# Lcrypto/mod-interleaveavx_multithreads-FAID

Hardware: AMD Instinct MI355X
Metric: decoded Gb/s @ 10 iters, 50G-PON LDPC; FER match vs AVX512 ref (higher is better)
Workload: dtype i8

## Files before the change

include/lnsfaid.h:

```cpp
#ifndef LNSFAID_H
#define LNSFAID_H

#include <stddef.h>
#include <stdint.h>

#ifdef __cplusplus
extern "C" {
#endif

#define LNSFAID_GROUP 32

#define LNSFAID_OK 0
#define LNSFAID_E_INVAL (-1)
#define LNSFAID_E_CODE (-2)
#define LNSFAID_E_NOMEM (-3)
#define LNSFAID_E_HIP (-4)
#define LNSFAID_E_NODEVICE (-5)
#define LNSFAID_E_INTERNAL (-6)

typedef struct lnsfaid_code {
    int32_t n_var;
    int32_t n_check;
    int32_t n_edges;
    int32_t z;
    int32_t puncture_tail;
    int32_t nb_degres;
    const int32_t* deg;
    const int32_t* deg_rows;
    const uint16_t* pos_vn;
} lnsfaid_code;

typedef struct lnsfaid_cfg {
    int32_t decode_method;
    int32_t max_iteration;
    int32_t factor_1;
    int32_t factor_2;
    int32_t floor_err_count;
    int32_t floor_iter_thresh;
    int32_t ef_elimination;
    int32_t max_bf_iter;
    int32_t bf_L0;
    int32_t bf_L1;
    int32_t bf_alpha;
    int32_t bf_delta;
    int32_t regular_col_weight;
    int32_t hard2_threshold;
    int32_t bf_vote_cap;
    int8_t v2c_map[6][4][8];
    int8_t v2c_map_ef[6][4][8];
} lnsfaid_cfg;

typedef struct lnsfaid_group_stats {
    int32_t iterations;
    int32_t bf_iterations;
} lnsfaid_group_stats;

typedef struct lnsfaid_codeword_stats {
    int32_t iterations;
    int32_t bf_iterations;
    int32_t unsatisfied;
} lnsfaid_codeword_stats;

typedef struct lnsfaid_ctx lnsfaid_ctx;


int lnsfaid_code_50gpon(lnsfaid_code* code, uint16_t* pos_vn, int32_t* deg3, int32_t* deg_rows3);

int lnsfaid_cfg_default(lnsfaid_cfg* cfg, int32_t decode_method, int32_t max_iteration);

#define LNSFAID_TABLES_FAID3 0
#define LNSFAID_TABLES_FAID32 1
#define LNSFAID_TABLES_FAID2 2
int lnsfaid_cfg_table_preset(lnsfaid_cfg* cfg, int32_t preset);

int lnsfaid_cfg_ef_elimination(lnsfaid_cfg* cfg, int32_t mode);


int lnsfaid_create(lnsfaid_ctx** ctx, const lnsfaid_code* code, const lnsfaid_cfg* cfg,
                   int32_t device, size_t max_groups);
void lnsfaid_destroy(lnsfaid_ctx* ctx);

int lnsfaid_set_cfg(lnsfaid_ctx* ctx, const lnsfaid_cfg* cfg);


int lnsfaid_decode(lnsfaid_ctx* ctx, const int8_t* fixInput, size_t n_groups,
                   int8_t* decodedBits, lnsfaid_group_stats* stats);

int lnsfaid_decode_device(lnsfaid_ctx* ctx, const int8_t* d_fixInput, size_t n_groups,
                          int8_t* d_decodedBits, lnsfaid_group_stats* d_stats);

#define LNSFAID_STOP_GROUP 0
#define LNSFAID_STOP_CODEWORD 1
int lnsfaid_set_early_stop(lnsfaid_ctx* ctx, int32_t rule);
int lnsfaid_early_stop(const lnsfaid_ctx* ctx);
int lnsfaid_decode_codewords(lnsfaid_ctx* ctx, const int8_t* fixInput, size_t n_groups, int8_t* decodedBits,
                             lnsfaid_codeword_stats* cw_stats);
int lnsfaid_decode_codewords_device(lnsfaid_ctx* ctx, const int8_t* d_fixInput, size_t n_groups, int8_t* d_decodedBits,
                                    lnsfaid_codeword_stats* d_cw_stats);

int lnsfaid_count_errors(lnsfaid_ctx* ctx, const int8_t* decodedBits, const int8_t* inputBits,
                         size_t n_groups, uint64_t out[4]);
int lnsfaid_count_errors_device(lnsfaid_ctx* ctx, const int8_t* d_decodedBits,
                                const int8_t* d_inputBits, size_t n_groups, uint64_t out[4]);

int lnsfaid_decode_packed(lnsfaid_ctx* ctx, const uint8_t* llr4, size_t n_groups, uint32_t* bits, lnsfaid_group_stats* stats);
int lnsfaid_decode_packed_device(lnsfaid_ctx* ctx, const uint8_t* d_llr4, size_t n_groups, uint32_t* d_bits,
                                 lnsfaid_group_stats* d_stats);
int lnsfaid_decode_codewords_packed(lnsfaid_ctx* ctx, const uint8_t* llr4, size_t n_groups, uint32_t* bits,
                                    lnsfaid_codeword_stats* cw_stats);
int lnsfaid_decode_codewords_packed_device(lnsfaid_ctx* ctx, const uint8_t* d_llr4, size_t n_groups, uint32_t* d_bits,
                                           lnsfaid_codeword_stats* d_cw_stats);
int lnsfaid_count_errors_packed(lnsfaid_ctx* ctx, const uint32_t* bits, const uint8_t* msg, size_t n_groups, uint64_t out[4]);
int lnsfaid_count_errors_packed_device(lnsfaid_ctx* ctx, const uint32_t* d_bits, const uint8_t* d_msg, size_t n_groups,
                                       uint64_t out[4]);
int lnsfaid_pack_llr4(const int8_t* fixInput, size_t n_values, uint8_t* llr4);
int lnsfaid_unpack_bits(const uint32_t* bits, size_t n_bits, int8_t* decodedBits);
int lnsfaid_pack_bits(const int8_t* inputBits, size_t n_bits, uint8_t* packed);


int lnsfaid_frontend_device(lnsfaid_ctx* ctx, const uint32_t* seeds, const uint64_t* draws_before, size_t n_streams,
                            int32_t mod_type, float sigma, float scale, const int8_t* codeword, int8_t* d_fixInput);
int lnsfaid_frontend_device_states(lnsfaid_ctx* ctx, const uint32_t* states, const uint64_t* draws_before, size_t n_streams,
                                   int32_t mod_type, float sigma, float scale, const int8_t* codeword, int8_t* d_fixInput);
uint64_t lnsfaid_frontend_draws_per_group(const lnsfaid_ctx* ctx, int32_t mod_type);

int lnsfaid_frontend_set_exact(lnsfaid_ctx* ctx, int32_t exact);
int lnsfaid_frontend_fastpath_bounds(lnsfaid_ctx* ctx, double measured[2], double assumed[2]);

int lnsfaid_frontend_set_interleave(lnsfaid_ctx* ctx, int32_t interleave_mod_type);

int lnsfaid_frontend_set_frames(lnsfaid_ctx* ctx, const int8_t* outputBits, const int8_t* inputBits, size_t n_streams);
int lnsfaid_frontend_input_bits(lnsfaid_ctx* ctx, const int8_t** d_inputBits);

int lnsfaid_demap_device(lnsfaid_ctx* ctx, const float* d_rx, size_t n_groups, int32_t mod_type, float scale, int8_t* d_fixInput);
int lnsfaid_demap_packed_device(lnsfaid_ctx* ctx, const float* d_rx, size_t n_groups, int32_t mod_type, float scale, uint8_t* d_llr4);
int lnsfaid_demap_host(int32_t n_var, int32_t n_check, int32_t interleave_mod_type, const float* rx, size_t n_groups,
                       int32_t mod_type, float scale, int8_t* fixInput);
int lnsfaid_demap_packed_host(int32_t n_var, int32_t n_check, int32_t interleave_mod_type, const float* rx, size_t n_groups,
                              int32_t mod_type, float scale, uint8_t* llr4);


int lnsfaid_code_parity_inverse(const lnsfaid_code* code, uint8_t* circ, size_t bytes);

int lnsfaid_encode_device(lnsfaid_ctx* ctx, const int8_t* d_inputBits, size_t n_groups, int8_t* d_outputBits);
int lnsfaid_encode(lnsfaid_ctx* ctx, const int8_t* inputBits, size_t n_groups, int8_t* outputBits);

int lnsfaid_frontend_random_frames(lnsfaid_ctx* ctx, const uint64_t* keys, size_t n_streams);

int lnsfaid_io_buffers(lnsfaid_ctx* ctx, int8_t** d_fixInput, int8_t** d_decodedBits, lnsfaid_group_stats** d_stats);

int lnsfaid_host_register(void* ptr, size_t bytes);
int lnsfaid_host_unregister(void* ptr);

int lnsfaid_read_stats(lnsfaid_ctx* ctx, lnsfaid_group_stats* stats, size_t n_groups);

#define LNSFAID_COMM_ID_BYTES 128
int lnsfaid_comm_unique_id(uint8_t id[LNSFAID_COMM_ID_BYTES]);
int lnsfaid_comm_init(lnsfaid_ctx* ctx, int32_t n_ranks, int32_t rank, const uint8_t id[LNSFAID_COMM_ID_BYTES]);
int lnsfaid_comm_attach(lnsfaid_ctx* ctx, void* nccl_comm);
int lnsfaid_comm_destroy(lnsfaid_ctx* ctx);
int lnsfaid_allreduce_counters(lnsfaid_ctx* ctx, uint64_t counters[4]);

int lnsfaid_select_kernel(lnsfaid_ctx* ctx, int32_t rows_per_lane);
int lnsfaid_kernel_rows_per_lane(const lnsfaid_ctx* ctx);

int lnsfaid_select_waves(lnsfaid_ctx* ctx, int32_t waves_per_codeword);
int lnsfaid_kernel_waves(const lnsfaid_ctx* ctx);

#define LNSFAID_MSG_REGISTERS 1
#define LNSFAID_MSG_HBM 2
int lnsfaid_select_message_store(lnsfaid_ctx* ctx, int32_t where);
int lnsfaid_message_store(const lnsfaid_ctx* ctx);

#define LNSFAID_ZERO_SHIFT_ON 1
#define LNSFAID_ZERO_SHIFT_OFF 2
int lnsfaid_select_zero_shift(lnsfaid_ctx* ctx, int32_t mode);
int lnsfaid_zero_shift_groups(const lnsfaid_ctx* ctx, int32_t* groups, int32_t n);
int lnsfaid_code_zero_shift_order(const lnsfaid_code* code, int32_t* groups, int32_t* order);

int lnsfaid_kernel_residency(lnsfaid_ctx* ctx, int32_t* workgroups_per_cu, int32_t* lds_limit);


int lnsfaid_kernel_time(lnsfaid_ctx* ctx, double* out_ms, uint64_t* out_launches, int32_t reset);

void* lnsfaid_stream(lnsfaid_ctx* ctx);

const char* lnsfaid_strerror(int err);
const char* lnsfaid_last_hip_error(void);
const char* lnsfaid_version(void);

#ifdef __cplusplus
}
#endif
#endif
```

mod-interleaveavx_multithreads-faid_amd/csrc/lnsfaid_capi.hip:

```cpp
#include <hip/hip_runtime.h>

#include <dlfcn.h>
#include <rccl/rccl.h>

#include <cstdio>
#include <cstdlib>
#include <cstring>
#include <new>
#include <vector>

#include "lnsfaid_device.h"
#include "lnsfaid_quantise.h"
#include "lnsfaid_swar.h"

extern "C" hipError_t lf_launch_decode(int method, int uniform_w, const LfKernelArgs* args, size_t lds_bytes,
                                       hipStream_t stream);
extern "C" const void* lf_decode_func(int method, int uniform_w);
extern "C" int lf_decode_threads(void);
extern "C" const void* lf_decode4_func(int method, int ef, int rm);
extern "C" int lf_decode4_threads(void);
extern "C" hipError_t lf_launch_decode4(int method, int ef, int rm, const LfKernelArgs* args, size_t lds_bytes, hipStream_t stream);
extern "C" int lf_decode4_rm_layers(void);
extern "C" const void* lf_decode4cw_func(int method, int ef, int rm);
extern "C" hipError_t lf_launch_decode4cw(int method, int ef, int rm, const LfCwArgs* args, size_t lds_bytes, hipStream_t stream);
extern "C" const void* lf_decode4p_func(int method, int ef, int rm, int per_codeword);
extern "C" hipError_t lf_launch_decode4p(int method, int ef, int rm, const LfKernelArgs* args, size_t lds_bytes, hipStream_t stream);
extern "C" hipError_t lf_launch_decode4pcw(int method, int ef, int rm, const LfCwArgs* args, size_t lds_bytes, hipStream_t stream);
extern "C" hipError_t lf_launch_unpack_llr4(const uint8_t* d_llr4, int8_t* d_fix, size_t n_values, hipStream_t stream);
extern "C" hipError_t lf_launch_pack_bits(const int8_t* d_decoded, uint32_t* d_bits, size_t n_values, hipStream_t stream);
extern "C" hipError_t lf_launch_count_errors_packed(const uint32_t* d_bits, const uint32_t* d_msg, int n_var, int k_info, size_t n_cw,
                                                    unsigned long long* out, hipStream_t stream);
extern "C" int lf_decode4z_inst(int deg, int zg);
extern "C" const void* lf_decode4z_func(int method);
extern "C" hipError_t lf_launch_decode4z(int method, const LfKernelArgs* args, size_t lds_bytes, hipStream_t stream);
extern "C" const void* lf_decode5_func(int method);
extern "C" int lf_decode5_threads(void);
extern "C" hipError_t lf_launch_decode5(int method, const LfKernelArgs* args, size_t lds_bytes, hipStream_t stream);
extern "C" hipError_t lf_launch_count_errors(const int8_t* decoded, const int8_t* input_bits, int n_var, int k_info,
                                             size_t n_cw, unsigned long long* out, hipStream_t stream);

extern "C" hipError_t lf_launch_frontend(const uint32_t* d_seeds, const unsigned long long* d_draws, int n_streams, int mod_type,
                                         float sigma_ch, float scale, const int8_t* d_codeword, const int8_t* d_frames, int n_var,
                                         int n_check, int interleave, int fast, int8_t* d_fix, hipStream_t stream);
extern "C" hipError_t lf_launch_demap(const float* d_rx, size_t n_groups, int mod_type, float scale, int n_var, int n_check,
                                      int interleave, int packed, void* d_out, hipStream_t stream);
extern "C" hipError_t lf_frontend_fastpath_scan(double* d_out2, hipStream_t stream);
extern "C" void lf_frontend_fastpath_assumed(double* eps2);
extern "C" hipError_t lf_launch_encode(const LfDevCode* d_code, int n_check, const uint32_t* d_bsup, const uint32_t* d_bsup_off,
                                       const int8_t* d_in, const unsigned long long* d_keys, size_t n_groups, int8_t* d_out,
                                       int8_t* d_info, hipStream_t stream);

#include <atomic>
#include <chrono>
#include <condition_variable>
#include <mutex>
#include <thread>
struct LfCombiner;
static thread_local char g_hip_err[256] = "";
static std::atomic<int> g_live_contexts(0);
#define LF_SPIN_CONTEXTS 4
static bool sync_blocking()
{
    static const char* e = getenv("LNSFAID_SYNC");
    if (e && e[0] == 's') return false;
    if (e && e[0] == 'b') return true;
    return g_live_contexts.load(std::memory_order_relaxed) > LF_SPIN_CONTEXTS;
}

static int hip_fail(hipError_t e, const char* what)
{
    snprintf(g_hip_err, sizeof(g_hip_err), "%s: %s", what, hipGetErrorString(e));
    return LNSFAID_E_HIP;
}
#define HIP_TRY(call)                                      \
    do {                                                   \
        hipError_t e_ = (call);                            \
        if (e_ != hipSuccess) return hip_fail(e_, #call);  \
    } while (0)

#define LF_IO_CHUNKS 8
#define LF_MAX_CHAIN 6

struct lnsfaid_ctx {
    int device = 0;
    size_t max_groups = 0;
    LfDevCode hcode;
    LfDevCfg hcfg;
    int n_var = 0, n_check = 0, k_info = 0;
    size_t lds_bytes = 0;
    hipStream_t stream = nullptr;
    hipEvent_t ev0 = nullptr, ev1 = nullptr;
    hipEvent_t ev_chain[LF_MAX_CHAIN + 1] = {};
    hipEvent_t ev_block = nullptr;
    uint32_t slot_seen[LF_MAX_CHAIN] = {};
    int predicted_launches = 1;
    hipStream_t s_in = nullptr, s_out = nullptr;
    hipEvent_t ev_in[LF_IO_CHUNKS] = {};
    LfDevCode* d_code = nullptr;
    LfDevCfg* d_cfg = nullptr;
    int8_t* d_en = nullptr;
    uint4* d_rows = nullptr;
    uint32_t* d_bits = nullptr;
    LfLaneState* d_lane = nullptr;
    int32_t* d_status[2] = { nullptr, nullptr };
    uint32_t* d_remaining = nullptr;
    int32_t* d_live = nullptr;
    unsigned long long* d_counters = nullptr;
    uint32_t* h_remaining = nullptr;
    unsigned long long* h_counters = nullptr;
    int8_t* d_io_in = nullptr;
    int8_t* d_io_out = nullptr;
    lnsfaid_group_stats* d_io_stats = nullptr;
    lnsfaid_codeword_stats* d_io_cw_stats = nullptr;
    uint8_t* d_pk_in = nullptr;
    uint32_t* d_pk_out = nullptr;
    lnsfaid_group_stats* d_pk_stats = nullptr;
    int early_stop = LNSFAID_STOP_GROUP;
    int rows_per_lane = 0;
    int waves_per_cw = 0;
    int msg_store = 0;
    int zero_shift = 0;
    struct LfCombiner* comb = nullptr;
    int comb_slot = -1;
    const void* checked_fn[4] = {};
    int resident_wg[4] = {}, lds_wg[4] = {};
    void* comm = nullptr;
    bool comm_owned = false;
    unsigned long long* d_reduce = nullptr;
    double kernel_ms = 0.0;
    uint64_t kernel_launches = 0;
    uint32_t* d_fe_seeds = nullptr;
    unsigned long long* d_fe_draws = nullptr;
    int8_t* d_fe_codeword = nullptr;
    int8_t* d_fe_frames = nullptr;
    int8_t* d_fe_input = nullptr;
    size_t fe_frames_streams = 0;
    int fe_interleave = 1;
    int fe_exact = 0;
    int enc_state = 0;
    uint32_t* d_enc_sup = nullptr;
    uint32_t* d_enc_off = nullptr;
    unsigned long long* d_fe_keys = nullptr;
};

static int stream_wait(lnsfaid_ctx* ctx)
{
    if (sync_blocking()) {
        HIP_TRY(hipEventRecord(ctx->ev_block, ctx->stream));
        HIP_TRY(hipEventSynchronize(ctx->ev_block));
    } else {
        HIP_TRY(hipStreamSynchronize(ctx->stream));
    }
    return LNSFAID_OK;
}

static int weight_class(int w) { return w == 3 ? 0 : (w == 6 ? 1 : (w == 11 ? 2 : 3)); }

static int build_code(const lnsfaid_code* code, LfDevCode* out)
{
    memset(out, 0, sizeof(*out));
    if (!code || !code->pos_vn || !code->deg || !code->deg_rows) return LNSFAID_E_INVAL;
    const int Z = code->z, N = code->n_var, M = code->n_check, E = code->n_edges;
    if (Z != LF_Z) return LNSFAID_E_CODE;
    if (N <= 0 || M <= 0 || N % Z || M % Z || M >= N) return LNSFAID_E_CODE;
    const int nbr = M / Z, nbc = N / Z, K = N - M;
    if (nbr > LF_MAX_BR || nbc > LF_MAX_BC) return LNSFAID_E_CODE;
    if (K % 4 || M % 4 || N % LF_T) return LNSFAID_E_CODE;
    if (code->puncture_tail < 0 || code->puncture_tail > N) return LNSFAID_E_CODE;
    std::vector<int> row_deg;
    row_deg.reserve(M);
    long e_total = 0;
    for (int k = 0; k < code->nb_degres; ++k) {
        if (code->deg_rows[k] < 0 || code->deg[k] < 2 || code->deg[k] > LF_MAX_DEG) return LNSFAID_E_CODE;
        for (int i = 0; i < code->deg_rows[k]; ++i) { row_deg.push_back(code->deg[k]); e_total += code->deg[k]; }
    }
    if ((int)row_deg.size() != M || e_total != E) return LNSFAID_E_CODE;

    size_t e = 0;
    for (int br = 0; br < nbr; ++br) {
        const int deg = row_deg[(size_t)br * Z];
        out->deg[br] = deg;
        const uint16_t* row0 = code->pos_vn + e;
        for (int j = 0; j < 64; ++j) out->sbtab[br][j] = 0u;
        for (int j = 0; j < 32; ++j) out->sbplain[br][j] = 0u;
        int prev_cb = -1;
        for (int j = 0; j < deg; ++j) {
            const int cb = row0[j] / Z, sh = row0[j] % Z;
            if (row0[j] >= N || cb <= prev_cb) return LNSFAID_E_CODE;
            prev_cb = cb;
            out->circ[br][j].sb = (uint32_t)cb * (uint32_t)Z + (uint32_t)sh;
            out->sbtab[br][LF_JCODE_A(j)] = out->sbtab[br][LF_JCODE_B(j)] = out->circ[br][j].sb;
            out->sbplain[br][j] = (((uint32_t)cb * (uint32_t)Z) << 16) | (((uint32_t)sh) << 2);
            out->s4tab[br][j] = ((uint32_t)sh) << 2;
            out->cbtab[br][j] = (uint32_t)cb * (uint32_t)Z;
            if (out->col_weight[cb] >= LF_MAX_COLW) return LNSFAID_E_CODE;
            out->colcirc[cb][out->col_weight[cb]++] = (uint32_t)br | ((uint32_t)sh << 8);
        }
        for (int i = 0; i < Z; ++i) {
            if (row_deg[(size_t)br * Z + i] != deg) return LNSFAID_E_CODE;
            for (int j = 0; j < deg; ++j) {
                const uint32_t sb = out->circ[br][j].sb;
                const int want = (int)(sb / (uint32_t)Z * (uint32_t)Z + (sb % (uint32_t)Z + (uint32_t)i) % (uint32_t)Z);
                if (code->pos_vn[e + (size_t)i * deg + j] != want) return LNSFAID_E_CODE;
            }
        }
        e += (size_t)deg * Z;
        for (int j = 0; j < 32; ++j) out->zsbplain[br][j] = 0u;
        int n = 0;
        for (int zero = 1; zero >= 0; --zero)
            for (int j = 0; j < deg; ++j)
                if ((out->s4tab[br][j] == 0u) == (zero != 0)) {
                    out->zsbplain[br][n] = out->sbplain[br][j];
                    out->zs4tab[br][n] = out->s4tab[br][j];
                    out->zcbtab[br][n] = out->cbtab[br][j];
                    ++n;
                }
        int n_zero = 0;
        while (n_zero < deg && out->zs4tab[br][n_zero] == 0u) ++n_zero;
        out->zinst[br] = lf_decode4z_inst(deg, n_zero / 4);
    }
    {
        const int nw = N / 32, pw = M / 32;
        const uint32_t hard0 = lf_lds_off_hard(N), zero = lf_lds_off_zero(N, nw, pw);
        if (lf_lds_bytes(N, nw, pw) > 0xffffu) return LNSFAID_E_CODE;
        for (int br = 0; br < LF_MAX_BR; ++br)
            for (int j = 0; j < LF_MAX_DEG; ++j)
                for (int k = 0; k < 8; ++k) {
                    uint2 e; e.x = zero | (zero << 16); e.y = 0;
                    if (br < nbr && j < out->deg[br]) {
                        const uint32_t sb = out->circ[br][j].sb, cb = sb / (uint32_t)Z, sh = sb % (uint32_t)Z;
                        const uint32_t o = (32u * (uint32_t)k + sh) & 255u, q = o >> 5;
                        e.x = (hard0 + 4u * (cb * 8u + q)) | ((hard0 + 4u * (cb * 8u + ((q + 1u) & 7u))) << 16);
                        e.y = o & 31u;
                    }
                    out->synw[br][j][k] = e;
                }
    }
    for (int br = 0; br < nbr; ++br)
        for (int j = 0; j < out->deg[br]; ++j)
            out->circ[br][j].wclass = (uint32_t)weight_class(out->col_weight[out->circ[br][j].sb / (uint32_t)Z]);
    out->n_var = N; out->n_check = M; out->k_info = K; out->nbr = nbr; out->nbc = nbc;
    out->puncture_tail = code->puncture_tail;
    out->n_words = N / 32; out->p_words = M / 32;
    return LNSFAID_OK;
}

static void build_wcols(LfDevCode* code, int W)
{
    code->n_wcols = 0;
    for (int cb = 0; cb < code->nbc; ++cb)
        if (code->col_weight[cb] == W) code->wcol[code->n_wcols++] = cb;
    bool seen[LF_MAX_BC] = {};
    for (int br = 0; br < LF_MAX_BR; ++br) {
        code->era_edges[br] = 0;
        for (int j = 0; br < code->nbr && j < code->deg[br]; ++j) {
            const int cb = (int)(code->circ[br][j].sb / LF_Z);
            if (code->col_weight[cb] == W && !seen[cb]) { seen[cb] = true; code->era_edges[br] |= 1u << j; }
        }
    }
}

static int build_cfg(const lnsfaid_cfg* cfg, LfDevCfg* out)
{
    if (!cfg) return LNSFAID_E_INVAL;
    if (cfg->decode_method < 0 || cfg->decode_method > 5) return LNSFAID_E_INVAL;
    if (cfg->max_iteration < 0 || cfg->max_iteration > (1 << 20)) return LNSFAID_E_INVAL;
    if (cfg->max_bf_iter < 0 || cfg->max_bf_iter > (1 << 20)) return LNSFAID_E_INVAL;
    if (cfg->regular_col_weight < 0 || cfg->regular_col_weight > LF_MAX_COLW) return LNSFAID_E_INVAL;
    memset(out, 0, sizeof(*out));
    out->method = cfg->decode_method;
    out->max_iter = cfg->max_iteration;
    out->factor_1 = cfg->decode_method == 0 ? (int16_t)cfg->factor_1 : (int8_t)cfg->factor_1;
    out->factor_2 = cfg->decode_method == 0 ? (int16_t)cfg->factor_2 : (int8_t)cfg->factor_2;
    out->floor_err_count = cfg->floor_err_count;
    out->floor_iter_thresh = cfg->floor_iter_thresh;
    out->ef = cfg->ef_elimination;
    out->max_bf = (cfg->decode_method == 0 || cfg->decode_method == 1) ? 0 : cfg->max_bf_iter;
    out->L0 = cfg->bf_L0; out->L1 = cfg->bf_L1; out->alpha = cfg->bf_alpha; out->delta = cfg->bf_delta;
    out->W = cfg->regular_col_weight;
    out->hard2_thr = cfg->hard2_threshold;
    out->vote_cap = (int8_t)cfg->bf_vote_cap;
    if ((cfg->decode_method == 1 || cfg->decode_method == 3 || cfg->decode_method == 4)
        && ((int8_t)cfg->factor_1 < 0 || (int8_t)cfg->factor_2 < 1)) return LNSFAID_E_INVAL;
    if (cfg->decode_method == 5 && cfg->ef_elimination != 1) return LNSFAID_E_INVAL;
    if (cfg->decode_method == 2 && (cfg->ef_elimination < 0 || cfg->ef_elimination > 2)) return LNSFAID_E_INVAL;
    if (cfg->decode_method != 2 && cfg->decode_method != 5 && cfg->ef_elimination != 0) return LNSFAID_E_INVAL;
    out->uniform_w = 1;
    for (int it = 0; it < 6; ++it)
        for (int w = 0; w < 4; ++w) {
            for (int a = 0; a < 8; ++a) {
                const int v = cfg->v2c_map[it][w][a], ve = cfg->v2c_map_ef[it][w][a];
                if ((cfg->decode_method == 2 || cfg->decode_method == 5) && (v < 0 || v > 7)) return LNSFAID_E_INVAL;
                if ((cfg->decode_method == 5 || cfg->ef_elimination >= 1) && (ve < 0 || ve > 7)) return LNSFAID_E_INVAL;
                uint32_t* l = a < 4 ? &out->lut_lo[it][w] : &out->lut_hi[it][w];
                uint32_t* le = a < 4 ? &out->lut_ef_lo[it][w] : &out->lut_ef_hi[it][w];
                *l |= (uint32_t)(v & 0xff) << (8 * (a & 3));
                *le |= (uint32_t)(ve & 0xff) << (8 * (a & 3));
                if (a > 0 && (v < cfg->v2c_map[it][w][a - 1] || ((cfg->decode_method == 5 || cfg->ef_elimination >= 1) && ve < cfg->v2c_map_ef[it][w][a - 1])))
                    out->uniform_w = 0;
            }
            if (out->lut_lo[it][w] != out->lut_lo[it][0] || out->lut_hi[it][w] != out->lut_hi[it][0]) out->uniform_w = 0;
            if ((cfg->decode_method == 5 || cfg->ef_elimination >= 1)
                && (out->lut_ef_lo[it][w] != out->lut_ef_lo[it][0] || out->lut_ef_hi[it][w] != out->lut_ef_hi[it][0]))
                out->uniform_w = 0;
        }
    if (cfg->decode_method == 0) {
        out->uniform_w = (out->factor_1 == out->factor_2) ? 1 : 0;
        out->nms_fits = sw_nms_fits(out->factor_1, out->factor_2) ? 1 : 0;
        if (out->nms_fits) sw_nms_tables(out->factor_1, out->nms_t);
    }
    if (cfg->decode_method == 2 && cfg->ef_elimination >= 1 && !out->uniform_w) return LNSFAID_E_INVAL;
    out->bf_fast = (out->W == 3 && ((int8_t)out->alpha == 0 || (int8_t)out->alpha == 1)) ? 1 : 0;
    return LNSFAID_OK;
}

static int check_code_for_method(const LfDevCode* code, int method)
{
    if (method == 3)
        for (int cb = 0; cb < code->nbc; ++cb)
            if (code->col_weight[cb] > 15) return LNSFAID_E_CODE;
    return LNSFAID_OK;
}

extern "C" int lnsfaid_comm_destroy(lnsfaid_ctx* ctx);
static int comb_join(lnsfaid_ctx* ctx);
static void comb_leave(lnsfaid_ctx* ctx, int slot);
extern "C" void lnsfaid_destroy(lnsfaid_ctx* ctx)
{
    if (!ctx) return;
    if (ctx->comb_slot >= 0) { comb_leave(ctx, ctx->comb_slot); ctx->comb_slot = -1; }
    g_live_contexts.fetch_sub(1, std::memory_order_relaxed);
    (void)hipSetDevice(ctx->device);
    if (ctx->stream) (void)hipStreamSynchronize(ctx->stream);
    (void)lnsfaid_comm_destroy(ctx);
    (void)hipFree(ctx->d_reduce);
    (void)hipFree(ctx->d_code); (void)hipFree(ctx->d_cfg); (void)hipFree(ctx->d_en); (void)hipFree(ctx->d_rows);
    (void)hipFree(ctx->d_bits); (void)hipFree(ctx->d_lane); (void)hipFree(ctx->d_status[0]); (void)hipFree(ctx->d_status[1]);
    (void)hipFree(ctx->d_remaining); (void)hipFree(ctx->d_live); (void)hipFree(ctx->d_counters);
    (void)hipFree(ctx->d_io_in); (void)hipFree(ctx->d_io_out); (void)hipFree(ctx->d_io_stats);
    (void)hipFree(ctx->d_io_cw_stats);
    (void)hipFree(ctx->d_pk_in); (void)hipFree(ctx->d_pk_out); (void)hipFree(ctx->d_pk_stats);
    (void)hipFree(ctx->d_fe_seeds); (void)hipFree(ctx->d_fe_draws); (void)hipFree(ctx->d_fe_codeword);
    (void)hipFree(ctx->d_fe_frames); (void)hipFree(ctx->d_fe_input);
    (void)hipFree(ctx->d_enc_sup); (void)hipFree(ctx->d_enc_off); (void)hipFree(ctx->d_fe_keys);
    if (ctx->h_remaining) (void)hipHostFree(ctx->h_remaining);
    if (ctx->h_counters) (void)hipHostFree(ctx->h_counters);
    if (ctx->ev0) (void)hipEventDestroy(ctx->ev0);
    if (ctx->ev1) (void)hipEventDestroy(ctx->ev1);
    for (auto e : ctx->ev_chain) if (e) (void)hipEventDestroy(e);
    if (ctx->ev_block) (void)hipEventDestroy(ctx->ev_block);
    if (ctx->stream) (void)hipStreamDestroy(ctx->stream);
    if (ctx->s_in) (void)hipStreamDestroy(ctx->s_in);
    if (ctx->s_out) (void)hipStreamDestroy(ctx->s_out);
    for (auto e : ctx->ev_in) if (e) (void)hipEventDestroy(e);
    delete ctx;
}

static int alloc_state(lnsfaid_ctx* ctx);
static int create_impl(lnsfaid_ctx* ctx, const lnsfaid_code* code, const lnsfaid_cfg* cfg)
{
    int rc = build_code(code, &ctx->hcode);
    if (rc) return rc;
    rc = build_cfg(cfg, &ctx->hcfg);
    if (rc) return rc;
    ctx->n_var = ctx->hcode.n_var; ctx->n_check = ctx->hcode.n_check; ctx->k_info = ctx->hcode.k_info;
    rc = check_code_for_method(&ctx->hcode, ctx->hcfg.method);
    if (rc) return rc;
    build_wcols(&ctx->hcode, ctx->hcfg.W);
    return alloc_state(ctx);
}

static int alloc_state(lnsfaid_ctx* ctx)
{
    ctx->n_var = ctx->hcode.n_var; ctx->n_check = ctx->hcode.n_check; ctx->k_info = ctx->hcode.k_info;
    ctx->lds_bytes = lf_lds_bytes(ctx->n_var, ctx->hcode.n_words, ctx->hcode.p_words);
    if (ctx->lds_bytes > 64 * 1024) return LNSFAID_E_CODE;

    int ndev = 0;
    if (hipGetDeviceCount(&ndev) != hipSuccess || ndev <= 0 || ctx->device < 0 || ctx->device >= ndev) {
        snprintf(g_hip_err, sizeof(g_hip_err), "no usable HIP device (count %d, asked for %d)", ndev, ctx->device);
        return LNSFAID_E_NODEVICE;
    }
    HIP_TRY(hipSetDevice(ctx->device));
    HIP_TRY(hipStreamCreateWithFlags(&ctx->stream, hipStreamNonBlocking));
    HIP_TRY(hipEventCreate(&ctx->ev0));
    HIP_TRY(hipEventCreate(&ctx->ev1));
    const size_t n_cw = ctx->max_groups * LNSFAID_GROUP;
    HIP_TRY(hipMalloc(&ctx->d_code, sizeof(LfDevCode)));
    HIP_TRY(hipMalloc(&ctx->d_cfg, sizeof(LfDevCfg)));
    HIP_TRY(hipMalloc(&ctx->d_en, n_cw * (size_t)ctx->n_var));
    HIP_TRY(hipMalloc(&ctx->d_rows, n_cw * (size_t)ctx->hcode.nbr * LF_T * sizeof(uint4)));
    HIP_TRY(hipMalloc(&ctx->d_bits, n_cw * (size_t)3 * ctx->hcode.n_words * sizeof(uint32_t)));
    HIP_TRY(hipMalloc(&ctx->d_lane, n_cw * sizeof(LfLaneState)));
    HIP_TRY(hipMalloc(&ctx->d_status[0], n_cw * sizeof(int32_t)));
    HIP_TRY(hipMalloc(&ctx->d_status[1], n_cw * sizeof(int32_t)));
    HIP_TRY(hipMalloc(&ctx->d_remaining, LF_MAX_CHAIN * sizeof(uint32_t)));
    HIP_TRY(hipMemset(ctx->d_remaining, 0, LF_MAX_CHAIN * sizeof(uint32_t)));
    for (auto& e : ctx->ev_chain) HIP_TRY(hipEventCreate(&e));
    HIP_TRY(hipEventCreateWithFlags(&ctx->ev_block, hipEventBlockingSync | hipEventDisableTiming));
    HIP_TRY(hipMalloc(&ctx->d_live, n_cw * sizeof(int32_t)));
    HIP_TRY(hipMalloc(&ctx->d_counters, 4 * sizeof(unsigned long long)));
    HIP_TRY(hipHostMalloc((void**)&ctx->h_remaining, LF_MAX_CHAIN * sizeof(uint32_t), hipHostMallocDefault));
    HIP_TRY(hipHostMalloc((void**)&ctx->h_counters, 4 * sizeof(unsigned long long), hipHostMallocDefault));
    HIP_TRY(hipMemcpy(ctx->d_code, &ctx->hcode, sizeof(LfDevCode), hipMemcpyHostToDevice));
    HIP_TRY(hipMemcpy(ctx->d_cfg, &ctx->hcfg, sizeof(LfDevCfg), hipMemcpyHostToDevice));
    return LNSFAID_OK;
}

extern "C" int lnsfaid_create(lnsfaid_ctx** out, const lnsfaid_code* code, const lnsfaid_cfg* cfg, int32_t device,
                              size_t max_groups)
{
    if (!out || !code || !cfg || max_groups == 0 || max_groups > ((size_t)1 << 24)) return LNSFAID_E_INVAL;
    *out = nullptr;
    lnsfaid_ctx* ctx = new (std::nothrow) lnsfaid_ctx();
    if (!ctx) return LNSFAID_E_NOMEM;
    ctx->device = device;
    ctx->max_groups = max_groups;
    if (const char* e = getenv("LNSFAID_ROWS_PER_LANE"))
        ctx->rows_per_lane = (e[0] == '2') ? 2 : 0;
    if (const char* e = getenv("LNSFAID_WAVES_PER_CODEWORD"))
        ctx->waves_per_cw = (e[0] == '2') ? 2 : 0;
    if (const char* e = getenv("LNSFAID_FRONTEND_EXACT"))
        ctx->fe_exact = (e[0] == '1') ? 1 : 0;
    if (const char* e = getenv("LNSFAID_MSG_STORE"))
        ctx->msg_store = (e[0] == 'h') ? LNSFAID_MSG_HBM : ((e[0] == 'r') ? LNSFAID_MSG_REGISTERS : 0);
    if (const char* e = getenv("LNSFAID_ZERO_SHIFT"))
        ctx->zero_shift = (e[0] == 'o' && e[1] == 'f') ? LNSFAID_ZERO_SHIFT_OFF : 0;
    g_live_contexts.fetch_add(1, std::memory_order_relaxed);
    const int rc = create_impl(ctx, code, cfg);
    if (rc) { lnsfaid_destroy(ctx); return rc; }
    ctx->comb_slot = comb_join(ctx);
    *out = ctx;
    return LNSFAID_OK;
}

extern "C" int lnsfaid_set_cfg(lnsfaid_ctx* ctx, const lnsfaid_cfg* cfg)
{
    if (!ctx || !cfg) return LNSFAID_E_INVAL;
    LfDevCfg n;
    int rc = build_cfg(cfg, &n);
    if (rc) return rc;
    rc = check_code_for_method(&ctx->hcode, n.method);
    if (rc) return rc;
    if (memcmp(&n, &ctx->hcfg, sizeof(n)) == 0) return LNSFAID_OK;
    HIP_TRY(hipSetDevice(ctx->device));
    HIP_TRY(hipStreamSynchronize(ctx->stream));
    if (n.W != ctx->hcfg.W) {
        build_wcols(&ctx->hcode, n.W);
        HIP_TRY(hipMemcpy(ctx->d_code, &ctx->hcode, sizeof(LfDevCode), hipMemcpyHostToDevice));
    }
    ctx->hcfg = n;
    HIP_TRY(hipMemcpy(ctx->d_cfg, &ctx->hcfg, sizeof(LfDevCfg), hipMemcpyHostToDevice));
    return LNSFAID_OK;
}

static void apply_devcfg(lnsfaid_ctx* ctx, const LfDevCfg& n)
{
    (void)hipStreamSynchronize(ctx->stream);
    ctx->hcfg = n;
    (void)hipMemcpy(ctx->d_cfg, &ctx->hcfg, sizeof(LfDevCfg), hipMemcpyHostToDevice);
}

static bool kernel4_possible(const lnsfaid_ctx* ctx)
{
    const int m = ctx->hcfg.method;
    if (m < 0 || m > 5) return false;
    if (m == 0) return ctx->hcfg.nms_fits != 0;
    if ((m == 2 || m == 5) && !ctx->hcfg.uniform_w) return false;
    return true;
}
static bool use_kernel4(const lnsfaid_ctx* ctx)
{
    if (ctx->hcfg.method == 2 && ctx->hcfg.ef >= 1) return true;
    if (ctx->rows_per_lane == 2) return false;
    return kernel4_possible(ctx);
}

extern "C" int lnsfaid_select_kernel(lnsfaid_ctx* ctx, int32_t rows_per_lane)
{
    if (!ctx || (rows_per_lane != 0 && rows_per_lane != 2 && rows_per_lane != 4)) return LNSFAID_E_INVAL;
    if (rows_per_lane == 4 && !kernel4_possible(ctx)) return LNSFAID_E_INVAL;
    if (rows_per_lane == 2 && ctx->hcfg.method == 2 && ctx->hcfg.ef >= 1) return LNSFAID_E_INVAL;
    ctx->rows_per_lane = rows_per_lane;
    return LNSFAID_OK;
}

extern "C" int lnsfaid_kernel_rows_per_lane(const lnsfaid_ctx* ctx) { return ctx ? (use_kernel4(ctx) ? 4 : 2) : LNSFAID_E_INVAL; }

static bool kernel5_possible(const lnsfaid_ctx* ctx)
{
    const int m = ctx->hcfg.method;
    return kernel4_possible(ctx) && m >= 1 && m <= 5 && !(m == 2 && ctx->hcfg.ef == 2) && ctx->hcode.n_words >= 7 * 64;
}
static bool use_kernel5(const lnsfaid_ctx* ctx) { return ctx->waves_per_cw == 2 && use_kernel4(ctx) && kernel5_possible(ctx); }

extern "C" int lnsfaid_select_waves(lnsfaid_ctx* ctx, int32_t waves_per_codeword)
{
    if (!ctx || waves_per_codeword < 0 || waves_per_codeword > 2) return LNSFAID_E_INVAL;
    if (waves_per_codeword == 2 && !(use_kernel4(ctx) && kernel5_possible(ctx))) return LNSFAID_E_INVAL;
    ctx->waves_per_cw = waves_per_codeword;
    return LNSFAID_OK;
}

extern "C" int lnsfaid_kernel_waves(const lnsfaid_ctx* ctx) { return ctx ? (use_kernel5(ctx) ? 2 : 1) : LNSFAID_E_INVAL; }

static bool msg_registers_possible(const lnsfaid_ctx* ctx)
{
    if (ctx->hcfg.method == 0) return false;
    return ctx->hcode.nbr <= lf_decode4_rm_layers() && !(ctx->hcfg.method == 2 && ctx->hcfg.ef == 2);
}
static bool use_msg_registers(const lnsfaid_ctx* ctx)
{
    if (!msg_registers_possible(ctx) || use_kernel5(ctx)) return false;
    return ctx->msg_store != LNSFAID_MSG_HBM;
}

static int layer_zero_groups(const lnsfaid_ctx* ctx, int br) { return (ctx->hcode.zinst[br] >> 8) & 0xff; }
static bool zero_shift_possible(const lnsfaid_ctx* ctx)
{
    if (!use_kernel4(ctx) || use_kernel5(ctx) || !use_msg_registers(ctx)) return false;
    if (ctx->hcfg.method < 1 || ctx->hcfg.method > 5 || !lf_decode4z_func(ctx->hcfg.method)) return false;
    for (int br = 0; br < ctx->hcode.nbr; ++br)
        if (layer_zero_groups(ctx, br) >= 1) return true;
    return false;
}
static bool use_zero_shift(const lnsfaid_ctx* ctx) { return ctx->zero_shift != LNSFAID_ZERO_SHIFT_OFF && zero_shift_possible(ctx); }

extern "C" int lnsfaid_select_zero_shift(lnsfaid_ctx* ctx, int32_t mode)
{
    if (!ctx || mode < 0 || mode > LNSFAID_ZERO_SHIFT_OFF) return LNSFAID_E_INVAL;
    if (mode == LNSFAID_ZERO_SHIFT_ON && !zero_shift_possible(ctx)) return LNSFAID_E_INVAL;
    ctx->zero_shift = mode;
    return LNSFAID_OK;
}

extern "C" int lnsfaid_zero_shift_groups(const lnsfaid_ctx* ctx, int32_t* groups, int32_t n)
{
    if (!ctx || n < 0 || (n > 0 && !groups)) return LNSFAID_E_INVAL;
    const bool on = use_zero_shift(ctx);
    for (int br = 0; br < n; ++br) groups[br] = (on && br < ctx->hcode.nbr) ? layer_zero_groups(ctx, br) : 0;
    return on ? 1 : 0;
}

extern "C" int lnsfaid_code_zero_shift_order(const lnsfaid_code* code, int32_t* groups, int32_t* order)
{
    LfDevCode* dc = new (std::nothrow) LfDevCode;
    if (!dc) return LNSFAID_E_NOMEM;
    const int rc = build_code(code, dc);
    if (rc) { delete dc; return rc; }
    const int nbr = dc->nbr;
    for (int br = 0; br < nbr; ++br) {
        int n_zero = 0;
        while (n_zero < dc->deg[br] && dc->zs4tab[br][n_zero] == 0u) ++n_zero;
        if (groups) groups[br] = n_zero / 4;
        for (int j = 0; order && j < LF_MAX_DEG; ++j) {
            order[br * LF_MAX_DEG + j] = -1;
            for (int i = 0; j < dc->deg[br] && i < dc->deg[br]; ++i)
                if (dc->cbtab[br][i] == dc->zcbtab[br][j] && dc->s4tab[br][i] == dc->zs4tab[br][j]) order[br * LF_MAX_DEG + j] = i;
        }
    }
    delete dc;
    return nbr;
}

static bool cw_possible(const lnsfaid_ctx* ctx) { return ctx->waves_per_cw != 2 && use_kernel4(ctx); }

static bool packed_kernel(const lnsfaid_ctx* ctx) { return use_kernel4(ctx) && !use_kernel5(ctx); }

static const void* selected_kernel(const lnsfaid_ctx* ctx, int* threads, int rule, bool packed = false)
{
    if (packed) {
        *threads = lf_decode4_threads();
        return lf_decode4p_func(ctx->hcfg.method, ctx->hcfg.ef, use_msg_registers(ctx) ? 1 : 0, rule == LNSFAID_STOP_CODEWORD ? 1 : 0);
    }
    if (rule == LNSFAID_STOP_CODEWORD) {
        *threads = lf_decode4_threads();
        return cw_possible(ctx) ? lf_decode4cw_func(ctx->hcfg.method, ctx->hcfg.ef, use_msg_registers(ctx) ? 1 : 0) : nullptr;
    }
    if (use_kernel5(ctx)) {
        *threads = lf_decode5_threads();
        return lf_decode5_func(ctx->hcfg.method);
    }
    if (use_zero_shift(ctx)) {
        *threads = lf_decode4_threads();
        return lf_decode4z_func(ctx->hcfg.method);
    }
    if (use_kernel4(ctx)) {
        *threads = lf_decode4_threads();
        return lf_decode4_func(ctx->hcfg.method, ctx->hcfg.ef, use_msg_registers(ctx) ? 1 : 0);
    }
    *threads = lf_decode_threads();
    return lf_decode_func(ctx->hcfg.method, ctx->hcfg.uniform_w);
}

extern "C" int lnsfaid_select_message_store(lnsfaid_ctx* ctx, int32_t where)
{
    if (!ctx || where < 0 || where > LNSFAID_MSG_HBM) return LNSFAID_E_INVAL;
    if (where == LNSFAID_MSG_REGISTERS && !msg_registers_possible(ctx)) return LNSFAID_E_INVAL;
    ctx->msg_store = where;
    return LNSFAID_OK;
}

extern "C" int lnsfaid_message_store(const lnsfaid_ctx* ctx)
{
    if (!ctx) return LNSFAID_E_INVAL;
    if (!use_kernel4(ctx)) return LNSFAID_MSG_HBM;
    return use_msg_registers(ctx) ? LNSFAID_MSG_REGISTERS : LNSFAID_MSG_HBM;
}

static int kernel_check(lnsfaid_ctx* ctx, int rule, bool packed = false)
{
    int threads = 0;
    const void* fn = selected_kernel(ctx, &threads, rule, packed);
    if (!fn) return rule == LNSFAID_STOP_CODEWORD ? LNSFAID_E_INVAL : LNSFAID_E_INTERNAL;
    const int slot = rule + (packed ? 2 : 0);
    if (fn == ctx->checked_fn[slot]) return LNSFAID_OK;
    hipFuncAttributes at;
    HIP_TRY(hipFuncGetAttributes(&at, fn));
    if (at.sharedSizeBytes != 0) {
        snprintf(g_hip_err, sizeof(g_hip_err), "decode kernel has %zu bytes of static LDS: its En image would not start at LDS offset 0",
                 (size_t)at.sharedSizeBytes);
        return LNSFAID_E_INTERNAL;
    }
    int wg = 0;
    HIP_TRY(hipOccupancyMaxActiveBlocksPerMultiprocessor(&wg, fn, threads, ctx->lds_bytes));
    hipDeviceProp_t prop;
    HIP_TRY(hipGetDeviceProperties(&prop, ctx->device));
    const size_t lds_cu = prop.maxSharedMemoryPerMultiProcessor ? prop.maxSharedMemoryPerMultiProcessor : 160 * 1024;
    const size_t gran = 512;
    int by_lds = (int)(lds_cu / ((ctx->lds_bytes + gran - 1) / gran * gran));
    const int by_waves = 32 / ((threads + 63) / 64);
    if (by_lds > by_waves) by_lds = by_waves;
    ctx->checked_fn[slot] = fn; ctx->resident_wg[slot] = wg; ctx->lds_wg[slot] = by_lds;
    static const bool trace = getenv("LNSFAID_TRACE") != nullptr;
    if (trace)
        fprintf(stderr, "[lnsfaid] decode kernel: %d threads, %d VGPRs, %zu B LDS per workgroup, %d workgroups per CU (LDS alone: %d)%s\n",
                threads, at.numRegs, ctx->lds_bytes, wg, by_lds, wg < by_lds ? "  ** residency lost **" : "");
    return LNSFAID_OK;
}

extern "C" int lnsfaid_kernel_residency(lnsfaid_ctx* ctx, int32_t* workgroups_per_cu, int32_t* lds_limit)
{
    if (!ctx) return LNSFAID_E_INVAL;
    HIP_TRY(hipSetDevice(ctx->device));
    const int rc = kernel_check(ctx, ctx->early_stop);
    if (rc) return rc;
    if (workgroups_per_cu) *workgroups_per_cu = ctx->resident_wg[ctx->early_stop];
    if (lds_limit) *lds_limit = ctx->lds_wg[ctx->early_stop];
    return LNSFAID_OK;
}

static int decode_device_impl(lnsfaid_ctx* ctx, const int8_t* d_fixInput, size_t n_groups, int8_t* d_decodedBits,
                              lnsfaid_group_stats* d_stats, bool status_preloaded, bool packed = false);
static int decode_cw_device_impl(lnsfaid_ctx* ctx, const int8_t* d_fixInput, size_t n_groups, int8_t* d_decodedBits,
                                 lnsfaid_group_stats* d_stats, lnsfaid_codeword_stats* d_cw_stats, bool status_preloaded,
                                 bool packed = false);
static int decode_device_rule(lnsfaid_ctx* ctx, const int8_t* d_fixInput, size_t n_groups, int8_t* d_decodedBits, lnsfaid_group_stats* d_stats,
                              lnsfaid_codeword_stats* d_cw_stats, int rule, bool status_preloaded)
{
    if (rule == LNSFAID_STOP_CODEWORD)
        return decode_cw_device_impl(ctx, d_fixInput, n_groups, d_decodedBits, d_stats, d_cw_stats, status_preloaded);
    return decode_device_impl(ctx, d_fixInput, n_groups, d_decodedBits, d_stats, status_preloaded);
}
extern "C" int lnsfaid_decode_device(lnsfaid_ctx* ctx, const int8_t* d_fixInput, size_t n_groups, int8_t* d_decodedBits,
                                     lnsfaid_group_stats* d_stats)
{
    if (!ctx) return LNSFAID_E_INVAL;
    return decode_device_rule(ctx, d_fixInput, n_groups, d_decodedBits, d_stats, nullptr, ctx->early_stop, false);
}
extern "C" int lnsfaid_decode_codewords_device(lnsfaid_ctx* ctx, const int8_t* d_fixInput, size_t n_groups, int8_t* d_decodedBits,
                                               lnsfaid_codeword_stats* d_cw_stats)
{
    return decode_cw_device_impl(ctx, d_fixInput, n_groups, d_decodedBits, nullptr, d_cw_stats, false);
}

extern "C" int lnsfaid_set_early_stop(lnsfaid_ctx* ctx, int32_t rule)
{
    if (!ctx || (rule != LNSFAID_STOP_GROUP && rule != LNSFAID_STOP_CODEWORD)) return LNSFAID_E_INVAL;
    ctx->early_stop = rule;
    return LNSFAID_OK;
}
extern "C" int lnsfaid_early_stop(const lnsfaid_ctx* ctx) { return ctx ? ctx->early_stop : LNSFAID_E_INVAL; }

static int decode_cw_device_impl(lnsfaid_ctx* ctx, const int8_t* d_fixInput, size_t n_groups, int8_t* d_decodedBits,
                                 lnsfaid_group_stats* d_stats, lnsfaid_codeword_stats* d_cw_stats, bool status_preloaded, bool packed)
{
    if (!ctx || (n_groups && (!d_fixInput || !d_decodedBits))) return LNSFAID_E_INVAL;
    if (n_groups > ctx->max_groups) return LNSFAID_E_INVAL;
    if (!cw_possible(ctx)) return LNSFAID_E_INVAL;
    if (n_groups == 0) return LNSFAID_OK;
    HIP_TRY(hipSetDevice(ctx->device));
    {
        const int rc = kernel_check(ctx, LNSFAID_STOP_CODEWORD, packed);
        if (rc) return rc;
    }
    const size_t n_cw = n_groups * LNSFAID_GROUP;
    LfCwArgs a;
    a.code = ctx->d_code; a.cfg = ctx->d_cfg;
    a.fix_input = d_fixInput; a.decoded = d_decodedBits;
    a.st_rows = ctx->d_rows;
    a.skip = status_preloaded ? ctx->d_status[0] : nullptr;
    a.stats = d_stats; a.cw_stats = d_cw_stats; a.n_cw = (int32_t)n_cw;
    if (d_stats) HIP_TRY(hipMemsetAsync(d_stats, 0, n_groups * sizeof(lnsfaid_group_stats), ctx->stream));
    static const bool trace = getenv("LNSFAID_TRACE") != nullptr;
    HIP_TRY(hipEventRecord(ctx->ev_chain[0], ctx->stream));
    if (packed) HIP_TRY(lf_launch_decode4pcw(ctx->hcfg.method, ctx->hcfg.ef, use_msg_registers(ctx) ? 1 : 0, &a, ctx->lds_bytes, ctx->stream));
    else HIP_TRY(lf_launch_decode4cw(ctx->hcfg.method, ctx->hcfg.ef, use_msg_registers(ctx) ? 1 : 0, &a, ctx->lds_bytes, ctx->stream));
    HIP_TRY(hipEventRecord(ctx->ev_chain[1], ctx->stream));
    { const int rcw = stream_wait(ctx); if (rcw) return rcw; }
    float ms = 0.f;
    HIP_TRY(hipEventElapsedTime(&ms, ctx->ev_chain[0], ctx->ev_chain[1]));
    ctx->kernel_ms += ms;
    ctx->kernel_launches += 1;
    if (trace) fprintf(stderr, "[lnsfaid] per-codeword launch: %.3f ms, %zu codewords\n", ms, n_cw);
    return LNSFAID_OK;
}

static int decode_device_impl(lnsfaid_ctx* ctx, const int8_t* d_fixInput, size_t n_groups, int8_t* d_decodedBits,
                              lnsfaid_group_stats* d_stats, bool status_preloaded, bool packed)
{
    if (!ctx || (n_groups && (!d_fixInput || !d_decodedBits))) return LNSFAID_E_INVAL;
    if (n_groups > ctx->max_groups) return LNSFAID_E_INVAL;
    if (n_groups == 0) return LNSFAID_OK;
    HIP_TRY(hipSetDevice(ctx->device));
    {
        const int rc = kernel_check(ctx, LNSFAID_STOP_GROUP, packed);
        if (rc) return rc;
    }
    const size_t n_cw = n_groups * LNSFAID_GROUP;
#ifdef LF4_LIVE_PROOF
    HIP_TRY(hipMemsetAsync(ctx->d_live, 0, n_cw * sizeof(int32_t), ctx->stream));
#endif

    LfKernelArgs a;
    a.code = ctx->d_code; a.cfg = ctx->d_cfg;
    a.fix_input = d_fixInput; a.decoded = d_decodedBits;
    a.st_en = ctx->d_en; a.st_rows = ctx->d_rows; a.st_bits = ctx->d_bits; a.st_lane = ctx->d_lane;
    a.live = ctx->d_live; a.stats = d_stats; a.n_cw = (int32_t)n_cw;

    const long max_launches = 2L * ((long)ctx->hcfg.max_iter + ctx->hcfg.max_bf + 2) + 2 + LF_MAX_CHAIN;
    static const bool trace = getenv("LNSFAID_TRACE") != nullptr;
    int cur = 0;
    long launch = 0, needed = 0;
    bool done = false;
    while (!done) {
        if (launch >= max_launches) return LNSFAID_E_INTERNAL;
        int chain = launch == 0 ? ctx->predicted_launches : 1;
        if (chain < 1) chain = 1;
        if (chain > LF_MAX_CHAIN) chain = LF_MAX_CHAIN;
        for (int j = 0; j < chain; ++j) {
            a.status_cur = (launch + j == 0 && !status_preloaded) ? nullptr : ctx->d_status[cur];
            a.status_next = ctx->d_status[cur ^ 1];
            a.remaining = ctx->d_remaining + j;
            HIP_TRY(hipEventRecord(ctx->ev_chain[j], ctx->stream));
            if (packed) HIP_TRY(lf_launch_decode4p(ctx->hcfg.method, ctx->hcfg.ef, use_msg_registers(ctx) ? 1 : 0, &a, ctx->lds_bytes, ctx->stream));
            else if (use_kernel5(ctx)) HIP_TRY(lf_launch_decode5(ctx->hcfg.method, &a, ctx->lds_bytes, ctx->stream));
            else if (use_zero_shift(ctx)) HIP_TRY(lf_launch_decode4z(ctx->hcfg.method, &a, ctx->lds_bytes, ctx->stream));
            else if (use_kernel4(ctx)) HIP_TRY(lf_launch_decode4(ctx->hcfg.method, ctx->hcfg.ef, use_msg_registers(ctx) ? 1 : 0, &a, ctx->lds_bytes, ctx->stream));
            else HIP_TRY(lf_launch_decode(ctx->hcfg.method, ctx->hcfg.uniform_w, &a, ctx->lds_bytes, ctx->stream));
            cur ^= 1;
        }
        HIP_TRY(hipEventRecord(ctx->ev_chain[chain], ctx->stream));
        HIP_TRY(hipMemcpyAsync(ctx->h_remaining, ctx->d_remaining, (size_t)chain * sizeof(uint32_t), hipMemcpyDeviceToHost, ctx->stream));
        { const int rcw = stream_wait(ctx); if (rcw) return rcw; }
        for (int j = 0; j < chain; ++j) {
            const uint32_t left = ctx->h_remaining[j] - ctx->slot_seen[j];
            ctx->slot_seen[j] = ctx->h_remaining[j];
            float ms = 0.f;
            HIP_TRY(hipEventElapsedTime(&ms, ctx->ev_chain[j], ctx->ev_chain[j + 1]));
            ctx->kernel_ms += ms;
            ctx->kernel_launches += 1;
            if (trace) fprintf(stderr, "[lnsfaid] launch %ld: %.3f ms, %u codewords left%s\n", launch + j, ms, left, done ? " (queued ahead, batch already complete)" : "");
            if (!done && left == 0) { done = true; needed = launch + j + 1; }
        }
        launch += chain;
    }
    ctx->predicted_launches = (int)needed;
    return LNSFAID_OK;
}

static int ensure_io(lnsfaid_ctx* ctx)
{
    if (ctx->d_io_in) return LNSFAID_OK;
    const size_t bytes = ctx->max_groups * LNSFAID_GROUP * (size_t)ctx->n_var;
    HIP_TRY(hipMalloc(&ctx->d_io_in, bytes));
    HIP_TRY(hipMalloc(&ctx->d_io_out, bytes));
    HIP_TRY(hipMalloc(&ctx->d_io_stats, ctx->max_groups * sizeof(lnsfaid_group_stats)));
    return LNSFAID_OK;
}

#define LF_COMB_SLOTS 128
#define LF_COMB_QUIET_US 150
#define LF_COMB_WINDOW_US 1500
#define LF_COMB_DEVICES 16
#define LF_COMB_WORKERS 4
#define LF_COMB_MIN_MEMBERS 4
enum { LF_SLOT_FREE = 0, LF_SLOT_IDLE, LF_SLOT_PENDING, LF_SLOT_RUNNING, LF_SLOT_DONE };
struct LfSlot {
    int state = LF_SLOT_FREE;
    int rc = 0;
    LfDevCfg cfg;
    int rule = LNSFAID_STOP_GROUP;
    lnsfaid_group_stats stats;
};
struct LfCombiner {
    int device = 0;
    std::mutex m;
    std::condition_variable cv_work, cv_done;
    std::thread worker[LF_COMB_WORKERS];
    bool stop = false, dead = false;
    bool gathering = false;
    int running = 0;
    lnsfaid_ctx* pool[LF_COMB_WORKERS] = {};
    LfDevCode code;
    size_t group_bytes = 0;
    int8_t *h_in = nullptr, *h_out = nullptr;
    int8_t *d_in_map = nullptr, *d_out_map = nullptr;
    int32_t* h_status = nullptr;
    lnsfaid_group_stats* h_stats = nullptr;
    LfSlot slots[LF_COMB_SLOTS];
    int members = 0, pending = 0;
    char err[256] = "";
    uint64_t batches = 0, calls = 0;
    double gather_ms = 0, device_ms = 0;
};
static std::mutex g_comb_mutex;
static LfCombiner* g_comb[LF_COMB_DEVICES] = {};

static int comb_workers()
{
    static const int n = [] {
        const char* e = getenv("LNSFAID_COMB_WORKERS");
        const int v = e ? atoi(e) : 2;
        return v < 1 ? 1 : (v > LF_COMB_WORKERS ? LF_COMB_WORKERS : v);
    }();
    return n;
}

static int comb_batches()
{
    static const int v = [] {
        const char* e = getenv("LNSFAID_COMB_BATCHES");
        const int n = e ? atoi(e) : 0;
        return n > 64 ? 64 : n;
    }();
    return v > comb_workers() ? v : comb_workers();
}

static bool comb_enabled()
{
    static const char* e = getenv("LNSFAID_COALESCE");
    return !(e && e[0] == '0');
}

static void apply_devcfg(lnsfaid_ctx* ctx, const LfDevCfg& n);

static void comb_run_batch(LfCombiner* cb, int w, const int* batch, int nb)
{
    lnsfaid_ctx* P = cb->pool[w];
    int32_t* h_status = cb->h_status + (size_t)w * LF_COMB_SLOTS * LNSFAID_GROUP;
    lnsfaid_group_stats* h_stats = cb->h_stats + (size_t)w * LF_COMB_SLOTS;
    int rc = LNSFAID_OK;
    auto fail = [&](hipError_t e, const char* what) { if (rc == LNSFAID_OK && e != hipSuccess) rc = hip_fail(e, what); };
    int lo = LF_COMB_SLOTS, hi = -1;
    for (int i = 0; i < nb; ++i) { lo = batch[i] < lo ? batch[i] : lo; hi = batch[i] > hi ? batch[i] : hi; }
    const size_t n = (size_t)hi + 1;
    for (size_t g = 0; g < n; ++g) {
        bool active = false;
        for (int i = 0; i < nb; ++i) active = active || (size_t)batch[i] == g;
        for (int l = 0; l < LNSFAID_GROUP; ++l) h_status[g * LNSFAID_GROUP + l] = active ? 0 : LF_DONE;
    }
    fail(hipSetDevice(cb->device), "hipSetDevice");
    if (rc == LNSFAID_OK && memcmp(&P->hcfg, &cb->slots[batch[0]].cfg, sizeof(LfDevCfg)) != 0) apply_devcfg(P, cb->slots[batch[0]].cfg);
    const size_t gb = cb->group_bytes, span = (size_t)(hi - lo + 1);
    fail(hipMemcpyAsync(P->d_status[0], h_status, n * LNSFAID_GROUP * sizeof(int32_t), hipMemcpyHostToDevice, P->stream), "status upload");
    static const bool copy_mode = getenv("LNSFAID_COMB_COPY") != nullptr;
    const int8_t* k_in = cb->d_in_map;
    int8_t* k_out = cb->d_out_map;
    if (copy_mode || !k_in || !k_out) {
        fail(hipMemcpyAsync(P->d_io_in + (size_t)lo * gb, cb->h_in + (size_t)lo * gb, span * gb, hipMemcpyHostToDevice, P->stream), "fixInput upload");
        k_in = P->d_io_in; k_out = P->d_io_out;
    }
    if (rc == LNSFAID_OK) rc = decode_device_rule(P, k_in, n, k_out, P->d_io_stats, nullptr, cb->slots[batch[0]].rule, true);
    if (rc == LNSFAID_OK) {
        if (k_out == P->d_io_out)
            fail(hipMemcpyAsync(cb->h_out + (size_t)lo * gb, P->d_io_out + (size_t)lo * gb, span * gb, hipMemcpyDeviceToHost, P->stream), "decodedBits download");
        fail(hipMemcpyAsync(h_stats + lo, P->d_io_stats + lo, span * sizeof(lnsfaid_group_stats), hipMemcpyDeviceToHost, P->stream), "stats download");
        if (rc == LNSFAID_OK) rc = stream_wait(P);
    }
    std::lock_guard<std::mutex> lk(cb->m);
    if (rc != LNSFAID_OK) snprintf(cb->err, sizeof(cb->err), "%s", g_hip_err);
    for (int i = 0; i < nb; ++i) {
        LfSlot& s = cb->slots[batch[i]];
        s.rc = rc;
        s.stats = h_stats[batch[i]];
        s.state = LF_SLOT_DONE;
    }
    cb->running -= nb;
    cb->batches += 1; cb->calls += (uint64_t)nb;
    cb->cv_done.notify_all();
    cb->cv_work.notify_all();
}

static void comb_worker(LfCombiner* cb, int w)
{
    std::unique_lock<std::mutex> lk(cb->m);
    for (;;) {
        cb->cv_work.wait(lk, [&] { return cb->stop || (cb->pending > 0 && !cb->gathering); });
        if (cb->stop) break;
        cb->gathering = true;
        const auto t_first = std::chrono::steady_clock::now();
        const auto deadline = t_first + std::chrono::microseconds(LF_COMB_WINDOW_US);
        for (;;) {
            const int share = (cb->members + comb_batches() - 1) / comb_batches();
            if (cb->stop || cb->pending >= share || cb->pending + cb->running >= cb->members) break;
            const int seen = cb->pending, seen_running = cb->running;
            auto quiet = std::chrono::steady_clock::now() + std::chrono::microseconds(LF_COMB_QUIET_US);
            if (quiet > deadline) quiet = deadline;
            cb->cv_work.wait_until(lk, quiet, [&] { return cb->pending != seen || cb->running != seen_running || cb->stop; });
            if (cb->pending == seen && cb->running == seen_running) break;
        }
        if (cb->stop) { cb->gathering = false; break; }
        cb->gather_ms += std::chrono::duration<double, std::milli>(std::chrono::steady_clock::now() - t_first).count();
        int batch[LF_COMB_SLOTS], nb = 0;
        const int cap = cb->members > 8 * comb_workers() ? (cb->members + comb_batches() - 1) / comb_batches() : LF_COMB_SLOTS;
        const LfDevCfg* cfg = nullptr;
        int rule = LNSFAID_STOP_GROUP;
        for (int i = 0; i < LF_COMB_SLOTS && nb < cap; ++i) {
            LfSlot& s = cb->slots[i];
            if (s.state != LF_SLOT_PENDING) continue;
            if (!cfg) { cfg = &s.cfg; rule = s.rule; }
            if (memcmp(cfg, &s.cfg, sizeof(LfDevCfg)) != 0 || s.rule != rule) continue;
            s.state = LF_SLOT_RUNNING;
            batch[nb++] = i;
        }
        cb->pending -= nb;
        cb->running += nb;
        cb->gathering = false;
        cb->cv_work.notify_all();
        if (nb == 0) continue;
        if (!cb->pool[w]) {
            lk.unlock();
            int rc = LNSFAID_OK;
            lnsfaid_ctx* P = new (std::nothrow) lnsfaid_ctx();
            if (!P) rc = LNSFAID_E_NOMEM;
            if (!rc) {
                P->device = cb->device; P->max_groups = LF_COMB_SLOTS;
                P->hcode = cb->code; P->hcfg = cb->slots[batch[0]].cfg;
                g_live_contexts.fetch_add(1, std::memory_order_relaxed);
                rc = alloc_state(P);
                if (!rc) rc = ensure_io(P);
                if (rc) { lnsfaid_destroy(P); P = nullptr; }
            }
            lk.lock();
            if (rc) {
                cb->dead = true;
                for (int i = 0; i < nb; ++i) { cb->slots[batch[i]].rc = rc; cb->slots[batch[i]].state = LF_SLOT_DONE; }
                cb->running -= nb;
                cb->cv_done.notify_all();
                continue;
            }
            cb->pool[w] = P;
        }
        lk.unlock();
        const auto t_dev = std::chrono::steady_clock::now();
        comb_run_batch(cb, w, batch, nb);
        lk.lock();
        cb->device_ms += std::chrono::duration<double, std::milli>(std::chrono::steady_clock::now() - t_dev).count();
    }
}

static int comb_join(lnsfaid_ctx* ctx)
{
    if (!comb_enabled() || ctx->max_groups != 1 || ctx->device < 0 || ctx->device >= LF_COMB_DEVICES) return -1;
    std::lock_guard<std::mutex> g(g_comb_mutex);
    LfCombiner* cb = g_comb[ctx->device];
    if (!cb) {
        cb = new (std::nothrow) LfCombiner();
        if (!cb) return -1;
        cb->device = ctx->device;
        cb->code = ctx->hcode;
        cb->group_bytes = (size_t)LNSFAID_GROUP * (size_t)ctx->n_var;
        g_comb[ctx->device] = cb;
    }
    std::lock_guard<std::mutex> lk(cb->m);
    if (cb->dead || memcmp(&cb->code, &ctx->hcode, sizeof(LfDevCode)) != 0) return -1;
    if (cb->members >= 1 && !cb->h_in) {
        const size_t bytes = (size_t)LF_COMB_SLOTS * cb->group_bytes;
        if (hipSetDevice(cb->device) != hipSuccess
            || hipHostMalloc((void**)&cb->h_in, bytes, hipHostMallocMapped) != hipSuccess
            || hipHostMalloc((void**)&cb->h_out, bytes, hipHostMallocMapped) != hipSuccess
            || hipHostMalloc((void**)&cb->h_status, (size_t)LF_COMB_WORKERS * LF_COMB_SLOTS * LNSFAID_GROUP * sizeof(int32_t), hipHostMallocDefault) != hipSuccess
            || hipHostMalloc((void**)&cb->h_stats, (size_t)LF_COMB_WORKERS * LF_COMB_SLOTS * sizeof(lnsfaid_group_stats), hipHostMallocDefault) != hipSuccess) {
            (void)hipGetLastError();
            if (cb->h_in) (void)hipHostFree(cb->h_in);
            if (cb->h_out) (void)hipHostFree(cb->h_out);
            if (cb->h_status) (void)hipHostFree(cb->h_status);
            if (cb->h_stats) (void)hipHostFree(cb->h_stats);
            cb->h_in = cb->h_out = nullptr; cb->h_status = nullptr; cb->h_stats = nullptr;
            cb->dead = true;
            return -1;
        }
        if (hipHostGetDevicePointer((void**)&cb->d_in_map, cb->h_in, 0) != hipSuccess
            || hipHostGetDevicePointer((void**)&cb->d_out_map, cb->h_out, 0) != hipSuccess) {
            (void)hipGetLastError();
            cb->d_in_map = cb->d_out_map = nullptr;
        }
        for (int w = 0; w < comb_workers(); ++w) cb->worker[w] = std::thread(comb_worker, cb, w);
    }
    for (int i = 0; i < LF_COMB_SLOTS; ++i)
        if (cb->slots[i].state == LF_SLOT_FREE) { cb->slots[i].state = LF_SLOT_IDLE; cb->members += 1; ctx->comb = cb; return i; }
    return -1;
}

static void comb_leave(lnsfaid_ctx* ctx, int slot)
{
    LfCombiner* cb = nullptr;
    {
        std::lock_guard<std::mutex> g(g_comb_mutex);
        cb = ctx->comb;
        if (!cb) return;
        bool last;
        {
            std::lock_guard<std::mutex> lk(cb->m);
            cb->slots[slot].state = LF_SLOT_FREE;
            cb->members -= 1;
            last = cb->members == 0;
            if (last) cb->stop = true;
            cb->cv_work.notify_all();
        }
        if (!last) return;
        if (g_comb[cb->device] == cb) g_comb[cb->device] = nullptr;
    }
    for (auto& th : cb->worker) if (th.joinable()) th.join();
    static const bool trace = getenv("LNSFAID_TRACE") != nullptr;
    if (trace && cb->batches)
        fprintf(stderr, "[lnsfaid] call combiner of device %d: %llu calls in %llu batches (%.1f per batch); per batch %.3f ms gathering, %.3f ms copies + decode\n",
                cb->device, (unsigned long long)cb->calls, (unsigned long long)cb->batches, (double)cb->calls / (double)cb->batches,
                cb->gather_ms / (double)cb->batches, cb->device_ms / (double)cb->batches);
    for (auto P : cb->pool) if (P) lnsfaid_destroy(P);
    if (cb->h_in) { (void)hipHostFree(cb->h_in); (void)hipHostFree(cb->h_out); (void)hipHostFree(cb->h_status); (void)hipHostFree(cb->h_stats); }
    delete cb;
}

static int comb_decode(lnsfaid_ctx* ctx, const int8_t* fixInput, int8_t* decodedBits, lnsfaid_group_stats* stats, int rule, int* rc_out)
{
    if (ctx->comb_slot < 0 || ctx->rows_per_lane != 0 || ctx->msg_store != 0 || ctx->waves_per_cw != 0 || ctx->zero_shift != 0) return 0;
    LfCombiner* cb = ctx->comb;
    const int slot = ctx->comb_slot;
    {
        std::lock_guard<std::mutex> lk(cb->m);
        if (cb->dead || cb->members < LF_COMB_MIN_MEMBERS || !cb->h_in) return 0;
        if (memcmp(&cb->code, &ctx->hcode, sizeof(LfDevCode)) != 0) return 0;
    }
    memcpy(cb->h_in + (size_t)slot * cb->group_bytes, fixInput, cb->group_bytes);
    int rc;
    {
        std::unique_lock<std::mutex> lk(cb->m);
        LfSlot& s = cb->slots[slot];
// ... 841 lines not shown
```

mod-interleaveavx_multithreads-faid_amd/csrc/lnsfaid_swar.h:

```cpp
#ifndef LNSFAID_SWAR_H
#define LNSFAID_SWAR_H

#include <stdint.h>

#if defined(__HIPCC__)
#define SW_DEV 1
#define SW_FN __device__ __forceinline__
#define SW_HD __host__ __device__ __forceinline__
#else
#define SW_DEV 0
#define SW_FN static inline
#define SW_HD static inline
#endif

#define SW_MAX_DEG 24
#ifndef SW_ILP
#define SW_ILP 4
#endif

#if SW_DEV
#define SW_SCHED_FENCE() __builtin_amdgcn_sched_barrier(0)
#else
#define SW_SCHED_FENCE() ((void)0)
#endif

SW_FN uint32_t sw_perm(uint32_t s0, uint32_t s1, uint32_t sel)
{
#if SW_DEV
    return __builtin_amdgcn_perm(s0, s1, sel);
#else
    const uint64_t in = ((uint64_t)s0 << 32) | s1;
    uint32_t r = 0;
    for (int i = 0; i < 4; ++i) {
        const uint32_t s = (sel >> (8 * i)) & 0xffu;
        uint32_t b;
        if (s >= 13) b = 0xff;
        else if (s == 12) b = 0;
        else if (s >= 8) b = ((in >> (8 * (2 * (s - 8) + 1) + 7)) & 1u) ? 0xffu : 0u;
        else b = (uint32_t)(in >> (8 * s)) & 0xffu;
        r |= b << (8 * i);
    }
    return r;
#endif
}
SW_FN uint32_t sw_alignbyte(uint32_t s0, uint32_t s1, uint32_t s2)
{
#if SW_DEV
    return __builtin_amdgcn_alignbyte(s0, s1, s2);
#else
    const uint64_t in = ((uint64_t)s0 << 32) | s1;
    return (uint32_t)(in >> (8 * (s2 & 3u)));
#endif
}
template <int TT>
SW_FN uint32_t sw_bitop3(uint32_t a, uint32_t b, uint32_t c)
{
#if SW_DEV
    return __builtin_amdgcn_bitop3_b32(a, b, c, TT);
#else
    uint32_t r = 0;
    for (int m = 0; m < 8; ++m)
        if ((TT >> m) & 1) r |= ((m & 4) ? a : ~a) & ((m & 2) ? b : ~b) & ((m & 1) ? c : ~c);
    return r;
#endif
}
#define SW_TT_SEL 0xca
#define SW_TT_XOR3 0x96
#define SW_TT_AND3 0x80
#define SW_TT_ANDOR 0xea
#define SW_TT_NANDOR 0xae
#define SW_TT_A_AND_BORC 0xe0
#define SW_TT_XORAND 0x28
#define SW_TT_BFI_C 0xd8
#define SW_TT_ANDNOT_OR 0xf8
#define SW_TT_XNOR_AND 0x82

SW_FN uint32_t sw_vconst(uint32_t k, uint32_t dep = 0u)
{
#if SW_DEV
    uint32_t r;
    asm("v_mov_b32 %0, %1 ; %2" : "=v"(r) : "s"(k), "s"(dep));
    return r;
#else
    (void)dep;
    return k;
#endif
}

#define SW_T2N_LO 0xf900fafbu
#define SW_T2N_HI 0xf8000000u

struct SwK {
    uint32_t c78, c0642, cfc, sel_sign, tt_lo, tt_hi, oh_lo, oh_hi;
    uint32_t cbit[8];
    uint32_t c7f;
    uint32_t c70;
    uint32_t n_lo, n_hi;
    uint32_t c55, c33, c0f;
    uint32_t cm27;
};
SW_FN SwK sw_consts(uint32_t dep = 0u)
{
    SwK k;
    k.c78 = sw_vconst(0x78787878u, dep); k.c0642 = sw_vconst(0x06040200u, dep); k.cfc = sw_vconst(0xfcu, dep);
    k.sel_sign = sw_vconst(0x0b090a08u, dep);
    k.tt_lo = sw_vconst(0x07030100u, dep); k.tt_hi = sw_vconst(0xff3f1f0fu, dep);
    k.oh_lo = sw_vconst(0x08040201u, dep); k.oh_hi = sw_vconst(0x80402010u, dep);
    for (int e = 0; e < 8; ++e) k.cbit[e] = sw_vconst(0x01010101u << e, dep);
    k.c7f = sw_vconst(0x7f7f7f7fu, dep);
    k.c70 = sw_vconst(0x70707070u, dep);
    k.n_lo = sw_vconst(SW_T2N_LO, dep); k.n_hi = sw_vconst(SW_T2N_HI, dep);
    k.c55 = sw_vconst(0x55555555u, dep); k.c33 = sw_vconst(0x33333333u, dep); k.c0f = sw_vconst(0x0f0f0f0fu, dep);
    k.cm27 = sw_vconst(0u - 0x27272727u, dep);
    return k;
}

SW_FN uint32_t sw_mask7(uint32_t x, uint32_t sel_sign) { return sw_perm(x, x << 8, sel_sign); }
#define SW_SEL_SIGN 0x0b090a08u

SW_FN uint32_t sw_popcount7(uint32_t x)
{
    x &= 0x7f7f7f7fu;
    x = x - ((x >> 1) & 0x55555555u);
    x = (x & 0x33333333u) + ((x >> 2) & 0x33333333u);
    return (x + (x >> 4)) & 0x0f0f0f0fu;
}
SW_FN uint32_t sw_therm2num(uint32_t x, uint32_t n_lo, uint32_t n_hi)
{
    const uint32_t a = sw_perm(n_hi, n_lo, x & 0x0f0f0f0fu);
    const uint32_t b = sw_perm(n_hi, n_lo, (x >> 4) & 0x07070707u);
    return a ^ b;
}
SW_FN uint32_t sw_zero_mask(uint32_t x, uint32_t sel_sign) { return ~sw_mask7(x + 0x7f7f7f7fu, sel_sign); }

SW_FN uint32_t sw_gather4(uint32_t g0, uint32_t g1, uint32_t g2, uint32_t g3)
{
    const uint32_t lo = (g1 << 8) | g0, hi = (g3 << 8) | g2;
    return (hi << 16) | lo;
}
SW_FN uint32_t sw_opaque(uint32_t x)
{
#if SW_DEV
    asm("" : "+v"(x));
#endif
    return x;
}
SW_FN uint32_t sw_node_addr(uint32_t x) { return sw_perm(x, x, 0x0c0c0300u) | ((x >> 8) & 3u); }

SW_FN uint32_t sw_table_pick(uint32_t rowmask, uint32_t w_hi, uint32_t w_lo, uint32_t t_hi, uint32_t t_lo, uint32_t m)
{
    return sw_bitop3<SW_TT_SEL>(rowmask, sw_perm(w_hi, w_lo, m), sw_perm(t_hi, t_lo, m));
}
SW_FN uint32_t sw_word_pick(uint32_t nm3, uint32_t nm4, uint32_t x0, uint32_t x1, uint32_t x2)
{
    return sw_bitop3<SW_TT_SEL>(nm4, sw_bitop3<SW_TT_SEL>(nm3, x0, x1), x2);
}
SW_FN void sw_word_deal(uint32_t keep, uint32_t nm3, uint32_t nm4, uint32_t oh[3])
{
    oh[0] = sw_bitop3<SW_TT_AND3>(keep, nm3, nm4);
    oh[1] = sw_bitop3<0x20>(keep, nm3, nm4);
    oh[2] = keep & ~nm4;
}
SW_FN uint32_t sw_argmin_selector(uint32_t w, uint32_t oh8, uint32_t c7f, uint32_t c01, uint32_t c0642)
{
    return sw_bitop3<SW_TT_ANDOR>(((w & oh8) + c7f) >> 7, c01, c0642);
}

struct SwRow {
    uint32_t x[3];
    uint32_t cw;
    uint32_t pa[2];
};

struct SwParams {
    uint32_t lut_lo, lut_hi;
    uint32_t ef_lo, ef_hi;
    int32_t f1, f2;
    int32_t window;
    int32_t ef_tables;
    uint32_t nms_t[4];
    uint32_t oms_lo[2], oms_hi[2];
};

#if SW_DEV
struct SwLds {
    typedef __attribute__((address_space(3))) uint32_t lds_u32;
    typedef __attribute__((address_space(3))) uint8_t lds_u8;
    SW_FN uint32_t rd32(uint32_t a) const { return *(const lds_u32*)(size_t)a; }
    SW_FN void wr32(uint32_t a, uint32_t v) const { *(lds_u32*)(size_t)a = v; }
    SW_FN uint32_t rd8(uint32_t a) const { return *(const lds_u8*)(size_t)a; }
    SW_FN void wr8(uint32_t a, uint32_t v) const { *(lds_u8*)(size_t)a = (uint8_t)v; }
};
#else
struct SwLds {
    uint8_t* base;
    uint32_t rd32(uint32_t a) const { return (uint32_t)base[a] | ((uint32_t)base[a + 1] << 8) | ((uint32_t)base[a + 2] << 16) | ((uint32_t)base[a + 3] << 24); }
    void wr32(uint32_t a, uint32_t v) const { base[a] = (uint8_t)v; base[a + 1] = (uint8_t)(v >> 8); base[a + 2] = (uint8_t)(v >> 16); base[a + 3] = (uint8_t)(v >> 24); }
    uint32_t rd8(uint32_t a) const { return base[a]; }
    void wr8(uint32_t a, uint32_t v) const { base[a] = (uint8_t)v; }
};
#endif

#define SW_BIAS_EN 120

SW_FN uint32_t sw_en_pos(uint32_t v) { return (v & ~255u) | ((v & 63u) << 2) | ((v >> 6) & 3u); }

#define SW_OMS(M) ((M) == 1 || (M) == 3 || (M) == 4)
#define SW_MINSUM(M) ((M) == 0 || SW_OMS(M))

SW_FN int sw_oms_offset(int x, bool window, bool F, int f1, int f2)
{
    if (window && F) {
        if (x < f2) x += 1;
        if (x <= f1) x += 1;
    } else {
        if (x > f1) x -= 1;
        if (x >= f2) x -= 1;
    }
    return x;
}

SW_FN void sw_oms_tables(SwParams& p)
{
    for (int r = 0; r < 2; ++r) {
        uint32_t lo = 0, hi = 0;
        for (int x = 0; x < 8; ++x) {
            const int a = sw_oms_offset(x, r != 0, r != 0, p.f1, p.f2);
            const uint32_t v = (uint32_t)((a > 7 ? 7 : a) & 0xff);
            if (x < 4) lo |= v << (8 * x); else hi |= v << (8 * (x - 4));
        }
        p.oms_lo[r] = lo; p.oms_hi[r] = hi;
    }
}

SW_HD int sw_nms_cste(int m, int factor)
{
    const uint16_t p = (uint16_t)((uint16_t)m * (uint16_t)(int16_t)factor);
    const int16_t q = (int16_t)(p >> 5);
    const int r = q > 127 ? 127 : q;
    return r > 7 ? 7 : r;
}
SW_HD bool sw_nms_fits(int f1, int f2)
{
    if (f1 != f2) return false;
    for (int m = 1; m < 32; ++m)
        if (sw_nms_cste(m, f1) < sw_nms_cste(m - 1, f1)) return false;
    return sw_nms_cste(15, f1) == 7;
}
SW_HD void sw_nms_tables(int factor, uint32_t nms_t[4])
{
    for (int w = 0; w < 4; ++w) nms_t[w] = 0;
    for (int m = 0; m < 16; ++m) {
        const int c = sw_nms_cste(m, factor);
        const uint32_t code = c >= 7 ? 0xffu : ((1u << c) - 1u);
        nms_t[m >> 2] |= code << (8 * (m & 3));
    }
}

struct SwUpd {
    uint32_t za[2], sb[2];
    uint32_t oc[2], hi[2];
};
template <bool MINSUM, bool FLIP = true>
SW_FN SwUpd sw_update_consts(uint32_t c, uint32_t flip, uint32_t bias)
{
    const uint32_t za_p = 0x1f1f1f1fu - bias, za_n = za_p - c;
    const uint32_t sb_p = 0x27272727u - c, sb_n = 0x27272727u;
    const uint32_t oc_p = 0x3f3f3f3fu - c, oc_n = MINSUM ? 0x3f3f3f3fu : oc_p;
    const uint32_t hi_p = 0xbebebebeu - c, hi_n = MINSUM ? 0xbebebebeu : hi_p;
    SwUpd u;
    if (!FLIP) {
        u.za[1] = za_p; u.za[0] = za_n; u.sb[1] = sb_p; u.sb[0] = sb_n; u.oc[1] = oc_p; u.oc[0] = oc_n; u.hi[1] = hi_p; u.hi[0] = hi_n;
        return u;
    }
    u.za[1] = sw_bitop3<SW_TT_SEL>(flip, za_n, za_p); u.za[0] = sw_bitop3<SW_TT_SEL>(flip, za_p, za_n);
    u.sb[1] = sw_bitop3<SW_TT_SEL>(flip, sb_n, sb_p); u.sb[0] = sw_bitop3<SW_TT_SEL>(flip, sb_p, sb_n);
    if (MINSUM) {
        u.oc[1] = sw_bitop3<SW_TT_SEL>(flip, oc_n, oc_p); u.oc[0] = sw_bitop3<SW_TT_SEL>(flip, oc_p, oc_n);
        u.hi[1] = sw_bitop3<SW_TT_SEL>(flip, hi_n, hi_p); u.hi[0] = sw_bitop3<SW_TT_SEL>(flip, hi_p, hi_n);
    } else {
        u.oc[1] = u.oc[0] = oc_p; u.hi[1] = u.hi[0] = hi_p;
    }
    return u;
}
template <bool MINSUM>
SW_FN uint32_t sw_update(uint32_t tb, uint32_t ms, const SwUpd& u, uint32_t sel_sign, uint32_t c80)
{
    const uint32_t za = sw_bitop3<SW_TT_SEL>(ms, u.za[1], u.za[0]);
    const uint32_t sb = sw_bitop3<SW_TT_SEL>(ms, u.sb[1], u.sb[0]);
    const uint32_t oc = MINSUM ? sw_bitop3<SW_TT_SEL>(ms, u.oc[1], u.oc[0]) : u.oc[1];
    const uint32_t hi = MINSUM ? sw_bitop3<SW_TT_SEL>(ms, u.hi[1], u.hi[0]) : u.hi[1];
    const uint32_t zb = tb + za;
    const uint32_t mo = sw_mask7(zb - oc, sel_sign);
    const uint32_t mq = sw_mask7(zb, sel_sign);
    return sw_bitop3<SW_TT_SEL>(mo, hi, sw_bitop3<SW_TT_SEL>(mq, zb, c80)) - sb;
}

struct SwUpd2 {
    uint32_t c, fm, zc, oc, hi;
};
template <bool MINSUM>
SW_FN SwUpd2 sw_update2_consts(uint32_t c, uint32_t fm, uint32_t bias)
{
    SwUpd2 u;
    u.c = c; u.fm = fm;
    u.zc = 0x1f1f1f1fu - bias - c;
    u.oc = MINSUM ? 0u - 0x3f3f3f3fu : 0x3f3f3f3fu - c;
    u.hi = MINSUM ? 0xbebebebeu : 0xbebebebeu - c;
    return u;
}
SW_FN uint32_t sw_upd2_d(uint32_t ms, const SwUpd2& u) { return sw_bitop3<SW_TT_XORAND>(ms, u.fm, u.c); }
SW_FN uint32_t sw_upd2_zb(uint32_t tb, uint32_t d, const SwUpd2& u) { return tb + d + u.zc; }
template <bool MINSUM>
SW_FN uint32_t sw_upd2_out(uint32_t zb, uint32_t d, const SwUpd2& u)
{
    const uint32_t ov = MINSUM ? zb + d + u.oc : zb - u.oc;
    return sw_bitop3<0xcf>(zb, ov, ov);
}
template <bool MINSUM>
SW_FN uint32_t sw_upd2_limit(uint32_t ms, uint32_t d, const SwUpd2& u, uint32_t c80)
{
    return sw_bitop3<SW_TT_ANDOR>(ms, MINSUM ? u.hi - d : u.hi, c80);
}
SW_FN uint32_t sw_upd2_en(uint32_t mout, uint32_t lim, uint32_t zb, uint32_t d, uint32_t cm27) { return sw_bitop3<SW_TT_SEL>(mout, lim, zb) + d + cm27; }
template <bool MINSUM>
SW_FN uint32_t sw_update2(uint32_t tb, uint32_t ms, const SwUpd2& u, uint32_t sel_sign, uint32_t c80, uint32_t cm27)
{
    const uint32_t d = sw_upd2_d(ms, u);
    const uint32_t zb = sw_upd2_zb(tb, d, u);
    const uint32_t mout = sw_mask7(sw_upd2_out<MINSUM>(zb, d, u), sel_sign);
    return sw_upd2_en(mout, sw_upd2_limit<MINSUM>(ms, d, u, c80), zb, d, cm27);
}

SW_FN void sw_min_edge(uint32_t& t1, uint32_t& t2, uint32_t ta[5], uint32_t u, int j)
{
    t2 = sw_bitop3<SW_TT_A_AND_BORC>(t2, t1, u);
    t1 &= u;
#pragma unroll
    for (int b = 0; b < 5; ++b)
        if (((j >> b) & 1) == (b >= 3 ? 1 : 0)) ta[b] &= u;
}
SW_FN void sw_min_quad(uint32_t& t1, uint32_t& t2, uint32_t ta[5], uint32_t v0, uint32_t v1, uint32_t v2, uint32_t v3, int j0)
{
    const uint32_t p0 = v0 & v1, p1 = v2 & v3, q = p0 & p1;
    const uint32_t o0 = v0 | v1, o1 = v2 | v3;
    const uint32_t m2 = sw_bitop3<SW_TT_A_AND_BORC>(o0, p0, p1);
    const uint32_t y = sw_bitop3<SW_TT_A_AND_BORC>(t2, t1, q);
    t2 = sw_bitop3<SW_TT_AND3>(y, m2, o1);
    t1 &= q;
    ta[0] = sw_bitop3<SW_TT_AND3>(ta[0], v0, v2);
    ta[1] &= p0;
    if (((j0 >> 2) & 1) == 0) ta[2] &= q;
    if (((j0 >> 3) & 1) == 1) ta[3] &= q;
    if (((j0 >> 4) & 1) == 1) ta[4] &= q;
}

SW_FN void sw_sign_edge(uint32_t ns[3], uint32_t ms, int j, uint32_t cbit) { ns[j >> 3] = sw_bitop3<SW_TT_ANDNOT_OR>(ns[j >> 3], ms, cbit); }
template <int NJ>
SW_FN void sw_sign_quad(uint32_t ns[3], const uint32_t* ms, int j0, int deg, bool fixed, uint32_t c55, uint32_t c33, uint32_t c0f)
{
    uint32_t m[4];
#pragma unroll
    for (int g = 0; g < 4; ++g) m[g] = (j0 + g < NJ && (fixed || j0 + g < deg)) ? ms[j0 + g < NJ ? j0 + g : 0] : 0u;
    const bool has1 = j0 + 1 < NJ, has2 = j0 + 2 < NJ, has3 = j0 + 3 < NJ;
    const uint32_t a = has1 ? sw_bitop3<SW_TT_SEL>(c55, m[0], m[1]) : m[0];
    const uint32_t b = has3 ? sw_bitop3<SW_TT_SEL>(c55, m[2], m[3]) : m[2];
    const uint32_t q = has2 ? sw_bitop3<SW_TT_SEL>(c33, a, b) : a;
    ns[j0 >> 3] = (j0 & 4) ? sw_bitop3<SW_TT_SEL>(c0f, ns[j0 >> 3], q) : q;
}

SW_FN uint32_t sw_plane_bit(const SwLds& lds, uint32_t era_plane, uint32_t a)
{
    const uint32_t v = (a & ~255u) | ((a >> 2) & 63u) | ((a & 3u) << 6);
    return (lds.rd32(era_plane + ((v >> 5) << 2)) >> (v & 31u)) & 1u;
}

#if SW_DEV
#define SW_MFN __device__ __forceinline__
#else
#define SW_MFN inline
#endif
struct SwNoXch {
    SW_MFN void put(int, uint32_t) const {}
    SW_MFN uint32_t get(int) const { return 0u; }
    SW_MFN void barrier() const {}
};
#define SW_OWN(j) (WAVES == 1 || (((j) & 1) == WAVE))

template <int METHOD, int DEG, bool ERA = false, int WAVES = 1, int WAVE = 0, int ZG = 0, class Tab, class Xch = SwNoXch>
SW_FN SwRow sw_layer_step(const SwLds& lds, const Tab& tab, const SwParams& p, const SwK& K, uint32_t lane, int deg, SwRow cur, bool fresh,
                          uint32_t rowpar, bool lme, uint32_t era_edges = 0u, uint32_t era_plane = 0u, const Xch& xch = Xch())
{
    static_assert(WAVES == 1 || !ERA, "the erasing variant is built for one wave per codeword only");
    static_assert(!ERA || METHOD == 2, "the erasure exists in Decode_FAID only");
    static_assert(ZG == 0 || (DEG > 0 && WAVES == 1 && !ERA && SW_ILP * ZG <= DEG), "rotation-free groups: per-degree, one-wave, non-erasing instances");
    constexpr int NZ = SW_ILP * ZG;
    constexpr int NJ = DEG > 0 ? DEG : SW_MAX_DEG;
    constexpr bool MINSUM = SW_MINSUM(METHOD);
    constexpr bool QUADS = WAVES == 1 && SW_ILP == 4 && DEG > 0;
    constexpr bool NSTREE = WAVES == 1 && SW_ILP == 4;
    const uint32_t c01 = K.cbit[0], c80 = K.cbit[7], c7f = K.c7f, c78 = K.c78, c0642 = K.c0642, cfc = K.cfc, sel_sign = K.sel_sign;
    const uint32_t tid4 = lane << 2;
    uint32_t s4j[NJ], cbj[NJ];
#pragma unroll
    for (int j = 0; j < NJ; ++j) { s4j[j] = (DEG > 0 || j < deg) ? tab.s4(j) : 0u; cbj[j] = (DEG > 0 || j < deg) ? tab.cb256(j) : 0u; }

    const uint32_t c2o = cur.cw & 0x07070707u, c1o = (cur.cw >> 3) & 0x07070707u;
    const uint32_t kp = 0x08080808u - c2o, kn = 0x08080808u + c2o;
    const uint32_t bias = MINSUM ? 0u : 0x06040200u;
    const uint32_t kt_lo = sw_perm(kn, kp, 0x05010400u) + (MINSUM ? 0u : 0x02020000u), kt_hi = sw_perm(kn, kp, 0x07030602u) + (MINSUM ? 0u : 0x06060404u);
    const uint32_t tt_lo = K.tt_lo, tt_hi = K.tt_hi;

    uint32_t padd = 0, psub = 0;
#ifndef SW_EXP_NO_OLDPATCH
    if (!fresh && WAVE == 0) {
        const uint32_t a0 = cur.pa[0] & 0xffffu, a1 = cur.pa[0] >> 16, a2 = cur.pa[1] & 0xffffu, a3 = cur.pa[1] >> 16;
        SW_SCHED_FENCE();
        const uint32_t g0 = lds.rd8(a0), g1 = lds.rd8(a1), g2 = lds.rd8(a2), g3 = lds.rd8(a3);
        const uint32_t mneg = sw_mask7(cur.cw << 1, sel_sign);
        padd = sw_bitop3<SW_TT_SEL>(mneg, c1o, c2o); psub = sw_bitop3<SW_TT_SEL>(mneg, c2o, c1o);
        SW_SCHED_FENCE();
        const uint32_t r = sw_gather4(g0, g1, g2, g3) + padd - psub;
        const uint32_t rh = sw_opaque(r >> 8);
        lds.wr8(a0, r); lds.wr8(a1, rh); lds.wr8(a2, r >> 16); lds.wr8(a3, rh >> 16);
    }
#endif
    if (WAVES == 2) xch.barrier();

    SW_SCHED_FENCE();
    uint32_t tb[NJ], ts[NJ], ms[NJ], ad[NJ], rq[NJ], ld[NJ];
    uint32_t t1 = 0xffffffffu, t2 = 0xffffffffu, ta[5] = { 0xffffffffu, 0xffffffffu, 0xffffffffu, 0xffffffffu, 0xffffffffu };
    uint32_t sx = 0;

#pragma unroll
    for (int j = 0; j < NJ; ++j) {
        if (j < NZ) {
            ad[j] = tid4 | cbj[j];
        } else if ((DEG > 0 || j < deg) && SW_OWN(j)) {
            const uint32_t x4 = tid4 + s4j[j];
#if SW_DEV
            uint32_t a;
            asm("v_and_or_b32 %0, %1, %2, %3" : "=v"(a) : "v"(x4), "v"(cfc), "s"(cbj[j]));
#else
            const uint32_t a = (x4 & cfc) | cbj[j];
#endif
            ad[j] = a; rq[j] = x4 >> 8;
        }
    }
#pragma unroll
    for (int j = 0; j < NJ; ++j)
        if ((DEG > 0 || j < deg) && SW_OWN(j)) ld[j] = lds.rd32(ad[j]);
    SW_SCHED_FENCE();
#pragma unroll
    for (int j0 = 0; j0 < NJ; j0 += SW_ILP) {
        uint32_t r_[SW_ILP], x_[SW_ILP], s_[SW_ILP], k_[SW_ILP], a_[SW_ILP], i_[SW_ILP], u_[SW_ILP];
#define SW_EDGES(...) _Pragma("unroll") for (int g = 0; g < SW_ILP; ++g) { const int j = j0 + g; if (j < NJ && (DEG > 0 || j < deg) && SW_OWN(j)) { __VA_ARGS__ } }
        _Pragma("unroll") for (int g = SW_ILP - 1; g >= 0; --g) { const int j = j0 + g; if (j < NJ && (DEG > 0 || j < deg) && SW_OWN(j)) r_[g] = j < NZ ? ld[j] : sw_alignbyte(ld[j], ld[j], rq[j]); }
        SW_EDGES(x_[g] = (j & 7) ? cur.x[j >> 3] >> (j & 7) : cur.x[j >> 3];)
        SW_EDGES(s_[g] = sw_bitop3<SW_TT_ANDOR>(x_[g], c01, c0642);)
        SW_EDGES(k_[g] = sw_perm(kt_hi, kt_lo, s_[g]);)
        if (j0 < NZ) { _Pragma("unroll") for (int g = SW_ILP - 1; g >= 0; --g) tb[j0 + g] = r_[g] + k_[g]; }
        else { SW_EDGES(tb[j] = r_[g] + k_[g];) }
        if (ERA) {
            SW_EDGES(x_[g] &= c01;)
            SW_EDGES(
                if ((era_edges >> j) & 1u) {
                    uint32_t em = 0, match = 0;
                    _Pragma("unroll") for (int k = 0; k < 4; ++k) {
                        const uint32_t a = ad[j] + ((rq[j] + (uint32_t)k) & 3u);
                        em |= sw_plane_bit(lds, era_plane, a) ? (0xffu << (8 * k)) : 0u;
                        const uint32_t pold = (k & 1) ? cur.pa[k >> 1] >> 16 : cur.pa[k >> 1] & 0xffffu;
                        match |= (!fresh && a == pold) ? (0xffu << (8 * k)) : 0u;
                    }
                    const uint32_t en_true = r_[g] - (padd & match) + (psub & match);
                    const uint32_t neg01 = ~((en_true + 0x08080808u) >> 7) & c01;
                    tb[j] = sw_bitop3<SW_TT_SEL>(em, c80 + bias, tb[j]);
                    x_[g] = sw_bitop3<SW_TT_SEL>(em, neg01, x_[g]);
                })
        }
        SW_EDGES(ts[j] = MINSUM ? tb[j] : tb[j] - (ERA ? (x_[g] | c0642) : s_[g]);)
        SW_EDGES(ms[j] = sw_mask7(ts[j], sel_sign);)
        SW_EDGES(a_[g] = sw_bitop3<SW_TT_XOR3>(ts[j], c7f, ms[j]);)
        if (METHOD == 0) {
            uint32_t h_[SW_ILP];
            SW_EDGES(i_[g] = sw_bitop3<SW_TT_NANDOR>(ms[j], c01, K.c70);)
            SW_EDGES(a_[g] = (a_[g] + i_[g]) & 0x8f8f8f8fu;)
            SW_EDGES(h_[g] = sw_mask7(a_[g] << 4, sel_sign);)
            SW_EDGES(a_[g] &= 0x87878787u;)
            SW_EDGES(i_[g] = sw_perm(p.nms_t[3], p.nms_t[2], a_[g]);)
            SW_EDGES(u_[g] = sw_perm(p.nms_t[1], p.nms_t[0], a_[g]);)
            SW_EDGES(u_[g] = sw_bitop3<SW_TT_SEL>(h_[g], i_[g], u_[g]);)
        } else {
            SW_EDGES(i_[g] = MINSUM ? sw_bitop3<SW_TT_NANDOR>(ms[j], c01, c78) : sw_bitop3<SW_TT_XNOR_AND>(x_[g], ms[j], c01);)
            SW_EDGES(a_[g] = (MINSUM ? a_[g] + i_[g] : a_[g] + i_[g] + c78) & 0x87878787u;)
            SW_EDGES(u_[g] = sw_perm(tt_hi, tt_lo, a_[g]);)
        }
        SW_EDGES(
            if (WAVES == 2) sx ^= ts[j];
            else if (j & 1) sx = sw_bitop3<SW_TT_XOR3>(sx, ts[j - 1], ts[j]); else if (j == (DEG > 0 ? DEG : deg) - 1) sx ^= ts[j];)
        if (QUADS) {
            uint32_t v_[4];
            _Pragma("unroll") for (int g = 0; g < 4; ++g) v_[g] = j0 + g < NJ ? u_[g] : 0xffffffffu;
            sw_min_quad(t1, t2, ta, v_[0], v_[1], v_[2], v_[3], j0);
        } else {
            SW_EDGES(sw_min_edge(t1, t2, ta, u_[g], j);)
        }
    }

    if (WAVES == 2) {
        if (WAVE == 1) {
            xch.put(0, t1); xch.put(1, t2); xch.put(2, ta[1]); xch.put(3, ta[2]); xch.put(4, ta[3]); xch.put(5, ta[4]); xch.put(6, sx);
        }
        xch.barrier();
        if (WAVE == 0) {
            const uint32_t o1 = xch.get(0), o2 = xch.get(1);
            ta[0] = t1;
            t2 = sw_bitop3<SW_TT_AND3>(t2, o2, t1 | o1);
            t1 &= o1;
            ta[1] &= xch.get(2); ta[2] &= xch.get(3); ta[3] &= xch.get(4); ta[4] &= xch.get(5);
            sx ^= xch.get(6);
        }
    }
    uint32_t c2n_x = 0, fm_x = 0;
    if (WAVES == 2 && WAVE == 1) {
        xch.barrier();
        c2n_x = xch.get(0); fm_x = xch.get(1);
    }

    const uint32_t n_lo = WAVES == 2 ? SW_T2N_LO : K.n_lo, n_hi = WAVES == 2 ? SW_T2N_HI : K.n_hi;
    const uint32_t min1 = sw_therm2num(t1, n_lo, n_hi), min2 = sw_therm2num(t2, n_lo, n_hi);
    uint32_t c1n, c2n;
    if (METHOD == 0) {
        c2n = min1;
        c1n = min2;
    } else if (SW_OMS(METHOD)) {
        const bool win = p.window && lme;
        const uint32_t w_lo = win ? p.oms_lo[1] : p.oms_lo[0], w_hi = win ? p.oms_hi[1] : p.oms_hi[0];
        c2n = sw_table_pick(rowpar, w_hi, w_lo, p.oms_hi[0], p.oms_lo[0], min1);
        c1n = sw_table_pick(rowpar, w_hi, w_lo, p.oms_hi[0], p.oms_lo[0], min2);
    } else {
        const bool win = (METHOD == 5 || p.ef_tables) && p.window && lme;
        const uint32_t w_lo = win ? p.ef_lo : p.lut_lo, w_hi = win ? p.ef_hi : p.lut_hi;
        c2n = sw_table_pick(rowpar, w_hi, w_lo, p.lut_hi, p.lut_lo, min1);
        c1n = sw_table_pick(rowpar, w_hi, w_lo, p.lut_hi, p.lut_lo, min2);
    }
#if SW_DEV
    asm volatile("" : "+v"(c1n), "+v"(c2n));
#endif
    const uint32_t fm = (WAVES == 2 && WAVE == 1) ? fm_x : sw_mask7(sx, sel_sign);
    if (WAVES == 2 && WAVE == 1) { c2n = c2n_x; c1n = 0u; }

    uint32_t idx = 0, ne7_3 = 0, ne7_4 = 0;
#pragma unroll
    for (int b = 4; b >= 0; --b) {
        const uint32_t dd = sw_bitop3<SW_TT_XORAND>(ta[b], t1, c7f);
        const uint32_t ne7 = dd + c7f;
        const uint32_t ne = ne7 >> (7 - b);
        if (b == 4) ne7_4 = ne7;
        if (b == 3) ne7_3 = ne7;
        if (b == 4) idx = (DEG == 0 && deg <= 16) ? 0u : ~ne & (0x01010101u << 4);
        else if (b == 3) idx = (DEG == 0 && deg <= 8) ? idx : sw_bitop3<0xf2>(idx, ne | (idx >> 1), 0x01010101u << 3);
        else idx = sw_bitop3<SW_TT_ANDNOT_OR>(idx, ne, 0x01010101u << b);
    }

    uint32_t pa[4], sbk[4], gk0 = 0, gk1 = 0, gk2 = 0, gk3 = 0, xb = 0;
    const uint32_t idx4 = idx << 2;
#pragma unroll
#ifdef SW_EXP_NO_ARGMIN
    for (int k = 0; k < 4; ++k) sbk[k] = (cbj[k] << 16) | s4j[k];
#else
    for (int k = 0; k < 4; ++k) sbk[k] = WAVE == 0 ? tab.sb_dyn4((idx4 >> (8 * k)) & 0x7cu) : 0u;
#endif
    SW_SCHED_FENCE();

    const SwUpd2 u2 = sw_update2_consts<MINSUM>(c2n, fm, bias);
    const uint32_t cm27 = WAVES == 2 ? 0u - 0x27272727u : K.cm27;
    uint32_t ns[3] = { 0u, 0u, 0u };
    uint32_t cbit[8];
#pragma unroll
    for (int e = 0; e < 8; ++e) cbit[e] = K.cbit[e];
#define SW_PASS2_ARITH(J0, EN)                                                                                       \
    {                                                                                                                \
        const int j0 = (J0);                                                                                         \
        uint32_t d_[SW_ILP], zb[SW_ILP], mo[SW_ILP], lm[SW_ILP];                                                     \
        SW_EDGES(d_[g] = sw_upd2_d(ms[j], u2);)                                                                      \
        SW_EDGES(zb[g] = sw_upd2_zb(tb[j], d_[g], u2);)                                                              \
        SW_EDGES(mo[g] = sw_upd2_out<MINSUM>(zb[g], d_[g], u2);)                                                     \
        SW_EDGES(mo[g] = sw_mask7(mo[g], sel_sign);)                                              \
        SW_EDGES(lm[g] = sw_upd2_limit<MINSUM>(ms[j], d_[g], u2, c80);)                                              \
        SW_EDGES(EN[g] = sw_upd2_en(mo[g], lm[g], zb[g], d_[g], cm27);)                                              \
        SW_EDGES(if (j >= NZ) EN[g] = sw_alignbyte(EN[g], EN[g], 4u - rq[j]);)                                       \
        if (NSTREE) sw_sign_quad<NJ>(ns, ms, j0, deg, DEG > 0, K.c55, K.c33, K.c0f);                                 \
        else SW_EDGES(sw_sign_edge(ns, ms[j], j, cbit[j & 7]);)                                                      \
    }
#define SW_PASS2_STORE(J0, EN)                                                                                       \
    {                                                                                                                \
        const int j0 = (J0);                                                                                         \
        SW_EDGES(lds.wr32(ad[j], EN[g]);)                                                                            \
    }
    uint32_t en0[SW_ILP], en1[SW_ILP];
    SW_PASS2_ARITH(0, en0)
    SW_SCHED_FENCE();
#pragma unroll
    for (int k = 0; k < 4; ++k)
        pa[k] = sw_node_addr(tid4 + sbk[k] + ((uint32_t)k << 8));
#ifdef SW_EXP_NO_ARGMIN
    gk0 = ld[0] & 0xffu; gk1 = ld[1] & 0xffu; gk2 = ld[2] & 0xffu; gk3 = ld[3] & 0xffu;
#else
    if (WAVE == 0) { gk0 = lds.rd8(pa[0]); gk1 = lds.rd8(pa[1]); gk2 = lds.rd8(pa[2]); gk3 = lds.rd8(pa[3]); }
#endif
    if (WAVES == 2 && WAVE == 0) {
        xch.put(0, c2n); xch.put(1, fm);
        xch.barrier();
    }
    SW_SCHED_FENCE();
    SW_PASS2_STORE(0, en0)
    if (SW_ILP < NJ) { SW_PASS2_ARITH(SW_ILP, en1) SW_PASS2_STORE(SW_ILP, en1) }
    SW_SCHED_FENCE();
    const uint32_t oh8 = sw_perm(K.oh_hi, K.oh_lo, idx & 0x07070707u);
    const uint32_t nm4 = (DEG == 0 && deg <= 16) ? 0xffffffffu : sw_mask7(ne7_4, sel_sign);
    const uint32_t nm3 = (DEG == 0 && deg <= 8) ? 0xffffffffu : sw_mask7(ne7_3, sel_sign);
    const uint32_t selA = sw_argmin_selector(sw_word_pick(nm3, nm4, cur.x[0], cur.x[1], cur.x[2]), oh8, c7f, c01, c0642);
    if (ERA) xb = selA & c01;
    const uint32_t gb = sw_gather4(gk0, gk1, gk2, gk3);
    uint32_t tbA = gb + sw_perm(kt_hi, kt_lo, selA);
    if (ERA) {
        uint32_t em = 0, match = 0;
#pragma unroll
        for (int k = 0; k < 4; ++k) {
            const uint32_t ik = (idx >> (8 * k)) & 31u;
            if ((era_edges >> ik) & 1u) em |= sw_plane_bit(lds, era_plane, pa[k]) ? (0xffu << (8 * k)) : 0u;
            const uint32_t pold = (k & 1) ? cur.pa[k >> 1] >> 16 : cur.pa[k >> 1] & 0xffffu;
            match |= (!fresh && pa[k] == pold) ? (0xffu << (8 * k)) : 0u;
        }
        const uint32_t en_true = gb - (padd & match) + (psub & match);
        tbA = sw_bitop3<SW_TT_SEL>(em, c80 + bias, tbA);
        xb = sw_bitop3<SW_TT_SEL>(em, ~((en_true + 0x08080808u) >> 7) & c01, xb);
    }
    const uint32_t tsA = MINSUM ? tbA : tbA - (ERA ? (xb | c0642) : selA);
    const uint32_t msA = sw_mask7(tsA, sel_sign);
    const uint32_t negA = ~(msA ^ fm);
    const SwUpd2 u1 = sw_update2_consts<MINSUM>(c1n, fm, bias);
    const uint32_t enA = sw_update2<MINSUM>(tbA, msA, u1, sel_sign, c80, cm27);

#pragma unroll
    for (int jg = 2 * SW_ILP; jg < NJ; jg += SW_ILP) {
        uint32_t en[SW_ILP];
        SW_PASS2_ARITH(jg, en)
        SW_PASS2_STORE(jg, en)
    }
#undef SW_EDGES
#undef SW_PASS2_ARITH
#undef SW_PASS2_STORE
    if (WAVES == 2) {
        if (WAVE == 1) { xch.put(0, ns[0]); xch.put(1, ns[1]); xch.put(2, ns[2]); }
        xch.barrier();
        if (WAVE == 1) { SwRow none = { { 0u, 0u, 0u }, 0u, { 0u, 0u } }; return none; }
        ns[0] |= xch.get(0); ns[1] |= xch.get(1); ns[2] |= xch.get(2);
    }
#ifndef SW_EXP_NO_ARGMIN
    {
        const uint32_t eh = sw_opaque(enA >> 8);
        lds.wr8(pa[0], enA); lds.wr8(pa[1], eh); lds.wr8(pa[2], enA >> 16); lds.wr8(pa[3], eh >> 16);
    }
#endif

    SwRow out;
    const int n = DEG > 0 ? DEG : deg;
#pragma unroll
    for (int g = 0; g < 3; ++g) {
        const int cnt = n - 8 * g < 0 ? 0 : (n - 8 * g > 8 ? 8 : n - 8 * g);
        const uint32_t valid = 0x01010101u * ((1u << cnt) - 1u);
        out.x[g] = ~(ns[g] ^ fm) & valid;
    }
    if (!MINSUM) {
        const uint32_t z2 = sw_zero_mask(c2n, sel_sign), nz1 = ~sw_zero_mask(c1n, sel_sign);
        const uint32_t keep = oh8 & nz1;
        uint32_t oh[3];
        sw_word_deal(keep, nm3, nm4, oh);
#pragma unroll
        for (int g = 0; g < 3; ++g) out.x[g] &= ~z2 | oh[g];
    }
    out.cw = c2n | (c1n << 3) | (negA & 0x40404040u);
    out.pa[0] = pa[0] | (pa[1] << 16);
    out.pa[1] = pa[2] | (pa[3] << 16);
    return out;
}

#endif
```

mod-interleaveavx_multithreads-faid_amd/csrc/lnsfaid_tables.c:

```c
#include "lnsfaid.h"
#include <string.h>

#define GPON_Z 256
#define GPON_BLOCK_ROWS 12
#define GPON_BLOCK_COLS 69
#define GPON_MAX_DEG 23

typedef struct { int16_t cb; int16_t shift; } gpon_circ;

static const int gpon_row_deg[GPON_BLOCK_ROWS] = { 23, 22, 23, 23, 23, 23, 23, 23, 23, 23, 23, 23 };

static const gpon_circ gpon_base[GPON_BLOCK_ROWS][GPON_MAX_DEG] = {
     { {0,80}, {3,60}, {4,169}, {6,11}, {8,143}, {11,222}, {13,59}, {15,218}, {18,178}, {24,105}, {27,19}, {30,126}, {34,211}, {40,247}, {42,255}, {45,85}, {52,246}, {53,94}, {59,242}, {64,129}, {66,19}, {67,58}, {68,27} },
     { {1,0}, {3,0}, {5,0}, {7,0}, {9,0}, {11,0}, {13,0}, {15,0}, {17,0}, {18,0}, {20,0}, {24,0}, {27,0}, {32,0}, {36,0}, {39,0}, {43,0}, {47,0}, {52,0}, {56,0}, {60,0}, {67,0} },
     { {1,91}, {3,74}, {5,237}, {6,202}, {9,201}, {10,136}, {12,178}, {14,239}, {16,183}, {19,217}, {21,232}, {25,169}, {32,129}, {33,60}, {39,19}, {40,76}, {46,77}, {50,2}, {54,101}, {57,217}, {61,48}, {67,172}, {68,42} },
     { {0,105}, {3,87}, {5,43}, {7,165}, {9,180}, {11,80}, {12,227}, {14,221}, {16,77}, {19,0}, {24,16}, {29,252}, {31,96}, {33,0}, {38,17}, {44,219}, {47,198}, {48,165}, {53,36}, {58,171}, {63,228}, {67,39}, {68,234} },
     { {1,170}, {2,250}, {5,195}, {6,139}, {9,135}, {11,92}, {13,147}, {15,1}, {20,13}, {23,98}, {26,142}, {30,225}, {36,23}, {37,108}, {44,0}, {46,0}, {51,135}, {56,121}, {57,0}, {63,0}, {66,46}, {67,242}, {68,228} },
     { {1,46}, {3,37}, {5,49}, {6,150}, {8,65}, {11,177}, {12,144}, {14,70}, {16,95}, {19,221}, {23,192}, {25,128}, {28,214}, {34,51}, {38,100}, {41,19}, {44,235}, {52,4}, {55,251}, {58,109}, {64,140}, {67,193}, {68,241} },
     { {0,137}, {2,104}, {4,238}, {7,228}, {9,225}, {10,247}, {13,191}, {15,177}, {17,255}, {22,192}, {27,51}, {32,195}, {34,0}, {37,172}, {43,219}, {46,236}, {49,136}, {53,0}, {57,159}, {60,10}, {65,5}, {67,25}, {68,94} },
     { {1,118}, {2,15}, {4,93}, {7,228}, {9,78}, {11,16}, {12,0}, {14,48}, {16,0}, {20,62}, {22,0}, {25,0}, {30,0}, {36,112}, {38,0}, {45,0}, {49,0}, {50,0}, {55,22}, {61,0}, {62,0}, {67,120}, {68,192} },
     { {1,208}, {2,0}, {4,0}, {6,0}, {8,0}, {10,0}, {13,251}, {14,0}, {17,44}, {18,123}, {23,0}, {26,0}, {31,0}, {35,0}, {40,0}, {43,153}, {48,0}, {51,0}, {55,0}, {65,0}, {66,0}, {67,16}, {68,0} },
     { {0,0}, {3,123}, {5,41}, {6,191}, {8,211}, {10,217}, {12,243}, {14,97}, {16,252}, {21,0}, {28,0}, {31,41}, {35,29}, {37,0}, {42,0}, {47,193}, {49,145}, {54,0}, {61,140}, {62,46}, {65,58}, {67,202}, {68,215} },
     { {0,209}, {2,252}, {4,39}, {7,159}, {8,69}, {10,37}, {12,134}, {15,201}, {16,49}, {21,104}, {26,129}, {29,157}, {33,222}, {41,139}, {42,39}, {48,203}, {50,94}, {56,194}, {59,3}, {62,43}, {63,153}, {67,207}, {68,109} },
     { {0,53}, {2,93}, {4,216}, {7,57}, {8,9}, {10,130}, {13,130}, {15,238}, {22,144}, {28,162}, {29,0}, {35,175}, {39,145}, {41,0}, {45,36}, {51,91}, {54,22}, {58,0}, {59,0}, {60,212}, {64,0}, {67,69}, {68,88} },
};

int lnsfaid_code_50gpon(lnsfaid_code* code, uint16_t* pos_vn, int32_t* deg3, int32_t* deg_rows3)
{
    if (!code || !pos_vn || !deg3 || !deg_rows3) return LNSFAID_E_INVAL;
    size_t e = 0;
    for (int br = 0; br < GPON_BLOCK_ROWS; ++br)
        for (int i = 0; i < GPON_Z; ++i)
            for (int j = 0; j < gpon_row_deg[br]; ++j)
                pos_vn[e++] = (uint16_t)(gpon_base[br][j].cb * GPON_Z + ((gpon_base[br][j].shift + i) % GPON_Z));
    deg3[0] = 23; deg_rows3[0] = 256;
    deg3[1] = 22; deg_rows3[1] = 256;
    deg3[2] = 23; deg_rows3[2] = 2560;
    code->n_var = GPON_BLOCK_COLS * GPON_Z;
    code->n_check = GPON_BLOCK_ROWS * GPON_Z;
    code->n_edges = (int32_t)e;
    code->z = GPON_Z;
    code->puncture_tail = 384;
    code->nb_degres = 3;
    code->deg = deg3;
    code->deg_rows = deg_rows3;
    code->pos_vn = pos_vn;
    return LNSFAID_OK;
}

static void fill_map(int8_t dst[4][8], const int8_t row[8])
{
    for (int w = 0; w < 4; ++w) memcpy(dst[w], row, 8);
}

int lnsfaid_cfg_table_preset(lnsfaid_cfg* cfg, int32_t preset)
{
    static const int8_t faid3[6][8] = {
        { 0, 1, 1, 2, 3, 3, 3, 3 }, { 0, 1, 1, 2, 3, 3, 3, 3 }, { 0, 1, 1, 2, 4, 4, 4, 4 },
        { 0, 1, 1, 3, 3, 4, 4, 4 }, { 0, 1, 1, 3, 3, 3, 6, 6 }, { 0, 1, 1, 3, 3, 3, 7, 7 },
    };
    static const int8_t faid32[6][8] = {
        { 0, 1, 1, 2, 3, 3, 3, 3 }, { 0, 1, 1, 2, 3, 3, 3, 3 }, { 0, 1, 1, 2, 4, 4, 4, 4 },
        { 1, 1, 1, 1, 4, 4, 4, 4 }, { 1, 1, 1, 1, 5, 5, 5, 5 }, { 1, 1, 1, 1, 6, 6, 6, 6 },
    };
    static const int8_t faid2[6][8] = {
        { 0, 0, 2, 2, 2, 2, 2, 2 }, { 0, 0, 2, 2, 2, 2, 2, 2 }, { 1, 1, 1, 3, 3, 3, 3, 3 },
        { 1, 1, 1, 4, 4, 4, 4, 4 }, { 1, 1, 1, 5, 5, 5, 5, 5 }, { 1, 1, 1, 6, 6, 6, 6, 6 },
    };
    const int8_t (*t)[8] = preset == LNSFAID_TABLES_FAID3 ? faid3 : preset == LNSFAID_TABLES_FAID32 ? faid32
                         : preset == LNSFAID_TABLES_FAID2 ? faid2 : 0;
    if (!cfg || !t) return LNSFAID_E_INVAL;
    for (int it = 0; it < 6; ++it) fill_map(cfg->v2c_map[it], t[it]);
    return LNSFAID_OK;
}

int lnsfaid_cfg_default(lnsfaid_cfg* cfg, int32_t decode_method, int32_t max_iteration)
{
    static const int8_t faid3[6][8] = {
        { 0, 1, 1, 2, 3, 3, 3, 3 }, { 0, 1, 1, 2, 3, 3, 3, 3 }, { 0, 1, 1, 2, 4, 4, 4, 4 },
        { 0, 1, 1, 3, 3, 4, 4, 4 }, { 0, 1, 1, 3, 3, 3, 6, 6 }, { 0, 1, 1, 3, 3, 3, 7, 7 },
    };
    static const int8_t faid_2b1c[6][8] = {
        { 0, 0, 1, 2, 3, 3, 3, 3 }, { 0, 1, 1, 2, 3, 3, 3, 3 }, { 0, 1, 1, 2, 3, 3, 3, 3 },
        { 0, 1, 1, 3, 3, 4, 4, 4 }, { 0, 1, 1, 3, 3, 3, 6, 6 }, { 0, 1, 1, 3, 3, 3, 7, 7 },
    };
    static const int8_t ef[8] = { 2, 3, 3, 4, 5, 6, 6, 7 };
    static const int8_t ident[8] = { 0, 1, 2, 3, 4, 5, 6, 7 };

    if (!cfg || max_iteration < 0) return LNSFAID_E_INVAL;
    memset(cfg, 0, sizeof(*cfg));
    cfg->decode_method = decode_method;
    cfg->max_iteration = max_iteration;
    cfg->factor_1 = 1;
    cfg->factor_2 = 6;
    cfg->bf_L1 = 0;
    cfg->bf_alpha = 1;
    cfg->bf_delta = 1;
    cfg->regular_col_weight = 3;
    cfg->hard2_threshold = 13;
    cfg->bf_vote_cap = 5;
    for (int it = 0; it < 6; ++it) fill_map(cfg->v2c_map_ef[it], ef);
    switch (decode_method) {
    case 0:
        cfg->max_bf_iter = 0;
        for (int it = 0; it < 6; ++it) fill_map(cfg->v2c_map[it], ident);
        break;
    case 1:
        cfg->floor_err_count = 100;
        cfg->floor_iter_thresh = 4;
        cfg->ef_elimination = 0;
        cfg->max_bf_iter = 0;
        cfg->bf_L0 = 0;
        for (int it = 0; it < 6; ++it) fill_map(cfg->v2c_map[it], ident);
        break;
    case 3:
        cfg->floor_err_count = 100;
        cfg->floor_iter_thresh = 4;
        cfg->ef_elimination = 0;
        cfg->max_bf_iter = 50;
        for (int it = 0; it < 6; ++it) fill_map(cfg->v2c_map[it], ident);
        break;
    case 4:
        cfg->floor_err_count = 100;
        cfg->floor_iter_thresh = 4;
        cfg->ef_elimination = 0;
        cfg->max_bf_iter = 50;
        cfg->bf_L0 = 0;
        cfg->bf_L1 = 50;
        for (int it = 0; it < 6; ++it) fill_map(cfg->v2c_map[it], ident);
        break;
    case 2:
        cfg->floor_err_count = 0;
        cfg->floor_iter_thresh = -1;
        cfg->ef_elimination = 0;
        cfg->max_bf_iter = 10;
        cfg->bf_L0 = 50;
        for (int it = 0; it < 6; ++it) fill_map(cfg->v2c_map[it], faid3[it]);
        break;
    case 5:
        cfg->floor_err_count = 50;
        cfg->floor_iter_thresh = 6;
        cfg->ef_elimination = 1;
        cfg->max_bf_iter = 10;
        cfg->bf_L0 = 100;
        for (int it = 0; it < 6; ++it) fill_map(cfg->v2c_map[it], faid_2b1c[it]);
        break;
    default:
        return LNSFAID_E_INVAL;
    }
    return LNSFAID_OK;
}

int lnsfaid_cfg_ef_elimination(lnsfaid_cfg* cfg, int32_t mode)
{
    if (!cfg || cfg->decode_method != 2 || mode < 0 || mode > 2) return LNSFAID_E_INVAL;
    cfg->ef_elimination = mode;
    cfg->floor_err_count = mode == 0 ? 0 : (mode == 1 ? 100 : 20);
    cfg->floor_iter_thresh = mode == 0 ? -1 : 6;
    return LNSFAID_OK;
}
```

mod-interleaveavx_multithreads-faid_amd/pyabi.py:

```python
import ctypes as C
import os

HERE = os.path.dirname(os.path.abspath(__file__))
LIB_PATH = os.path.join(HERE, "csrc", "liblnsfaid.so")

GROUP = 32
MSG_REGISTERS, MSG_HBM = 1, 2
ZERO_SHIFT_ON, ZERO_SHIFT_OFF = 1, 2
STOP_GROUP, STOP_CODEWORD = 0, 1


class Code(C.Structure):
    _fields_ = [
        ("n_var", C.c_int32),
        ("n_check", C.c_int32),
        ("n_edges", C.c_int32),
        ("z", C.c_int32),
        ("puncture_tail", C.c_int32),
        ("nb_degres", C.c_int32),
        ("deg", C.POINTER(C.c_int32)),
        ("deg_rows", C.POINTER(C.c_int32)),
        ("pos_vn", C.POINTER(C.c_uint16)),
    ]


class Cfg(C.Structure):
    _fields_ = [
        ("decode_method", C.c_int32),
        ("max_iteration", C.c_int32),
        ("factor_1", C.c_int32),
        ("factor_2", C.c_int32),
        ("floor_err_count", C.c_int32),
        ("floor_iter_thresh", C.c_int32),
        ("ef_elimination", C.c_int32),
        ("max_bf_iter", C.c_int32),
        ("bf_L0", C.c_int32),
        ("bf_L1", C.c_int32),
        ("bf_alpha", C.c_int32),
        ("bf_delta", C.c_int32),
        ("regular_col_weight", C.c_int32),
        ("hard2_threshold", C.c_int32),
        ("bf_vote_cap", C.c_int32),
        ("v2c_map", C.c_int8 * 8 * 4 * 6),
        ("v2c_map_ef", C.c_int8 * 8 * 4 * 6),
    ]


class GroupStats(C.Structure):
    _fields_ = [("iterations", C.c_int32), ("bf_iterations", C.c_int32)]


class CodewordStats(C.Structure):
    _fields_ = [("iterations", C.c_int32), ("bf_iterations", C.c_int32), ("unsatisfied", C.c_int32)]


SYMBOLS = {
    "lnsfaid_code_50gpon": (C.c_int, [C.POINTER(Code), C.POINTER(C.c_uint16), C.POINTER(C.c_int32), C.POINTER(C.c_int32)]),
    "lnsfaid_cfg_default": (C.c_int, [C.POINTER(Cfg), C.c_int32, C.c_int32]),
    "lnsfaid_cfg_table_preset": (C.c_int, [C.POINTER(Cfg), C.c_int32]),
    "lnsfaid_cfg_ef_elimination": (C.c_int, [C.POINTER(Cfg), C.c_int32]),
    "lnsfaid_create": (C.c_int, [C.POINTER(C.c_void_p), C.POINTER(Code), C.POINTER(Cfg), C.c_int32, C.c_size_t]),
    "lnsfaid_destroy": (None, [C.c_void_p]),
    "lnsfaid_set_cfg": (C.c_int, [C.c_void_p, C.POINTER(Cfg)]),
    "lnsfaid_decode": (C.c_int, [C.c_void_p, C.c_void_p, C.c_size_t, C.c_void_p, C.c_void_p]),
    "lnsfaid_decode_device": (C.c_int, [C.c_void_p, C.c_void_p, C.c_size_t, C.c_void_p, C.c_void_p]),
    "lnsfaid_set_early_stop": (C.c_int, [C.c_void_p, C.c_int32]),
    "lnsfaid_early_stop": (C.c_int, [C.c_void_p]),
    "lnsfaid_decode_codewords": (C.c_int, [C.c_void_p, C.c_void_p, C.c_size_t, C.c_void_p, C.c_void_p]),
    "lnsfaid_decode_codewords_device": (C.c_int, [C.c_void_p, C.c_void_p, C.c_size_t, C.c_void_p, C.c_void_p]),
    "lnsfaid_count_errors": (C.c_int, [C.c_void_p, C.c_void_p, C.c_void_p, C.c_size_t, C.POINTER(C.c_uint64)]),
    "lnsfaid_count_errors_device": (C.c_int, [C.c_void_p, C.c_void_p, C.c_void_p, C.c_size_t, C.POINTER(C.c_uint64)]),
    "lnsfaid_decode_packed": (C.c_int, [C.c_void_p, C.c_void_p, C.c_size_t, C.c_void_p, C.c_void_p]),
    "lnsfaid_decode_packed_device": (C.c_int, [C.c_void_p, C.c_void_p, C.c_size_t, C.c_void_p, C.c_void_p]),
    "lnsfaid_decode_codewords_packed": (C.c_int, [C.c_void_p, C.c_void_p, C.c_size_t, C.c_void_p, C.c_void_p]),
    "lnsfaid_decode_codewords_packed_device": (C.c_int, [C.c_void_p, C.c_void_p, C.c_size_t, C.c_void_p, C.c_void_p]),
    "lnsfaid_count_errors_packed": (C.c_int, [C.c_void_p, C.c_void_p, C.c_void_p, C.c_size_t, C.POINTER(C.c_uint64)]),
    "lnsfaid_count_errors_packed_device": (C.c_int, [C.c_void_p, C.c_void_p, C.c_void_p, C.c_size_t, C.POINTER(C.c_uint64)]),
    "lnsfaid_pack_llr4": (C.c_int, [C.c_void_p, C.c_size_t, C.c_void_p]),
    "lnsfaid_unpack_bits": (C.c_int, [C.c_void_p, C.c_size_t, C.c_void_p]),
    "lnsfaid_pack_bits": (C.c_int, [C.c_void_p, C.c_size_t, C.c_void_p]),
    "lnsfaid_frontend_device": (C.c_int, [C.c_void_p, C.POINTER(C.c_uint32), C.POINTER(C.c_uint64), C.c_size_t, C.c_int32,
                                          C.c_float, C.c_float, C.c_void_p, C.c_void_p]),
    "lnsfaid_frontend_device_states": (C.c_int, [C.c_void_p, C.POINTER(C.c_uint32), C.POINTER(C.c_uint64), C.c_size_t, C.c_int32,
                                                 C.c_float, C.c_float, C.c_void_p, C.c_void_p]),
    "lnsfaid_frontend_draws_per_group": (C.c_uint64, [C.c_void_p, C.c_int32]),
    "lnsfaid_frontend_set_interleave": (C.c_int, [C.c_void_p, C.c_int32]),
    "lnsfaid_demap_device": (C.c_int, [C.c_void_p, C.c_void_p, C.c_size_t, C.c_int32, C.c_float, C.c_void_p]),
    "lnsfaid_demap_packed_device": (C.c_int, [C.c_void_p, C.c_void_p, C.c_size_t, C.c_int32, C.c_float, C.c_void_p]),
    "lnsfaid_demap_host": (C.c_int, [C.c_int32, C.c_int32, C.c_int32, C.c_void_p, C.c_size_t, C.c_int32, C.c_float, C.c_void_p]),
    "lnsfaid_demap_packed_host": (C.c_int, [C.c_int32, C.c_int32, C.c_int32, C.c_void_p, C.c_size_t, C.c_int32, C.c_float, C.c_void_p]),
    "lnsfaid_frontend_set_frames": (C.c_int, [C.c_void_p, C.c_void_p, C.c_void_p, C.c_size_t]),
    "lnsfaid_frontend_input_bits": (C.c_int, [C.c_void_p, C.POINTER(C.c_void_p)]),
    "lnsfaid_code_parity_inverse": (C.c_int, [C.POINTER(Code), C.c_void_p, C.c_size_t]),
    "lnsfaid_encode_device": (C.c_int, [C.c_void_p, C.c_void_p, C.c_size_t, C.c_void_p]),
    "lnsfaid_encode": (C.c_int, [C.c_void_p, C.c_void_p, C.c_size_t, C.c_void_p]),
    "lnsfaid_frontend_random_frames": (C.c_int, [C.c_void_p, C.POINTER(C.c_uint64), C.c_size_t]),
    "lnsfaid_io_buffers": (C.c_int, [C.c_void_p, C.POINTER(C.c_void_p), C.POINTER(C.c_void_p), C.POINTER(C.c_void_p)]),
    "lnsfaid_read_stats": (C.c_int, [C.c_void_p, C.c_void_p, C.c_size_t]),
    "lnsfaid_host_register": (C.c_int, [C.c_void_p, C.c_size_t]),
    "lnsfaid_host_unregister": (C.c_int, [C.c_void_p]),
    "lnsfaid_comm_unique_id": (C.c_int, [C.c_void_p]),
    "lnsfaid_comm_init": (C.c_int, [C.c_void_p, C.c_int32, C.c_int32, C.c_void_p]),
    "lnsfaid_comm_attach": (C.c_int, [C.c_void_p, C.c_void_p]),
    "lnsfaid_comm_destroy": (C.c_int, [C.c_void_p]),
    "lnsfaid_allreduce_counters": (C.c_int, [C.c_void_p, C.POINTER(C.c_uint64)]),
    "lnsfaid_select_kernel": (C.c_int, [C.c_void_p, C.c_int32]),
    "lnsfaid_kernel_rows_per_lane": (C.c_int, [C.c_void_p]),
    "lnsfaid_select_waves": (C.c_int, [C.c_void_p, C.c_int32]),
    "lnsfaid_frontend_set_exact": (C.c_int, [C.c_void_p, C.c_int32]),
    "lnsfaid_frontend_fastpath_bounds": (C.c_int, [C.c_void_p, C.POINTER(C.c_double), C.POINTER(C.c_double)]),
    "lnsfaid_kernel_waves": (C.c_int, [C.c_void_p]),
    "lnsfaid_select_message_store": (C.c_int, [C.c_void_p, C.c_int32]),
    "lnsfaid_message_store": (C.c_int, [C.c_void_p]),
    "lnsfaid_select_zero_shift": (C.c_int, [C.c_void_p, C.c_int32]),
    "lnsfaid_zero_shift_groups": (C.c_int, [C.c_void_p, C.POINTER(C.c_int32), C.c_int32]),
    "lnsfaid_code_zero_shift_order": (C.c_int, [C.POINTER(Code), C.POINTER(C.c_int32), C.POINTER(C.c_int32)]),
    "lnsfaid_kernel_residency": (C.c_int, [C.c_void_p, C.POINTER(C.c_int32), C.POINTER(C.c_int32)]),
    "lnsfaid_kernel_time": (C.c_int, [C.c_void_p, C.POINTER(C.c_double), C.POINTER(C.c_uint64), C.c_int32]),
    "lnsfaid_stream": (C.c_void_p, [C.c_void_p]),
    "lnsfaid_strerror": (C.c_char_p, [C.c_int]),
    "lnsfaid_last_hip_error": (C.c_char_p, []),
    "lnsfaid_version": (C.c_char_p, []),
}


def bind(lib, symbols):
    for name, (res, args) in symbols.items():
        fn = getattr(lib, name)
        fn.restype = res
        fn.argtypes = args
    return lib


_lib = None


def load():
    global _lib
    if _lib is None:
        if not os.path.exists(LIB_PATH):
            raise RuntimeError(
                "HIP extension %s is missing: run `python -c 'import __graft_entry__ as g; g.build()'` "
                "(no CPU fallback exists in the product path)" % LIB_PATH)
        _lib = bind(C.CDLL(LIB_PATH), SYMBOLS)
    return _lib


class Code50GPON:

    def __init__(self, lib=None):
        lib = lib or load()
        self.pos_vn = (C.c_uint16 * 70400)()
        self.deg = (C.c_int32 * 3)()
        self.deg_rows = (C.c_int32 * 3)()
        self.code = Code()
        rc = lib.lnsfaid_code_50gpon(C.byref(self.code), self.pos_vn, self.deg, self.deg_rows)
        if rc != 0:
            raise RuntimeError("lnsfaid_code_50gpon failed: %d" % rc)

    @property
    def N(self):
        return self.code.n_var

    @property
    def M(self):
        return self.code.n_check

    @property
    def K(self):
        return self.code.n_var - self.code.n_check


def code_zero_shift_order(code, lib=None):
    lib = lib or load()
    groups, order = (C.c_int32 * 32)(), (C.c_int32 * (32 * 24))()
    nbr = lib.lnsfaid_code_zero_shift_order(C.byref(code), groups, order)
    if nbr < 0:
        raise ValueError("lnsfaid_code_zero_shift_order failed: %d" % nbr)
    return list(groups[:nbr]), [[j for j in order[br * 24:br * 24 + 24] if j >= 0] for br in range(nbr)]


def default_cfg(method, max_iter, lib=None):
    lib = lib or load()
    cfg = Cfg()
    rc = lib.lnsfaid_cfg_default(C.byref(cfg), method, max_iter)
    if rc != 0:
        raise ValueError("lnsfaid_cfg_default(%d, %d) failed: %d" % (method, max_iter, rc))
    return cfg


def pack_llr4(fix_input, lib=None):
    import numpy as np
    lib = lib or load()
    fix_input = np.ascontiguousarray(fix_input, dtype=np.int8)
    out = np.empty(fix_input.size // 2, dtype=np.uint8)
    rc = lib.lnsfaid_pack_llr4(fix_input.ctypes.data, fix_input.size, out.ctypes.data)
    if rc != 0:
        raise ValueError("lnsfaid_pack_llr4 failed: %d" % rc)
    return out


def unpack_bits(bits, lib=None):
    import numpy as np
    lib = lib or load()
    bits = np.ascontiguousarray(bits, dtype=np.uint32)
    out = np.empty(bits.size * 32, dtype=np.int8)
    rc = lib.lnsfaid_unpack_bits(bits.ctypes.data, out.size, out.ctypes.data)
    if rc != 0:
        raise ValueError("lnsfaid_unpack_bits failed: %d" % rc)
    return out


def pack_bits(input_bits, lib=None):
    import numpy as np
    lib = lib or load()
    input_bits = np.ascontiguousarray(input_bits, dtype=np.int8)
    out = np.empty(input_bits.size // 8, dtype=np.uint8)
    rc = lib.lnsfaid_pack_bits(input_bits.ctypes.data, input_bits.size, out.ctypes.data)
    if rc != 0:
        raise ValueError("lnsfaid_pack_bits failed: %d" % rc)
    return out


def _demap_host(fn_name, packed, n_var, n_check, interleave, rx, n_groups, mod_type, scale, lib):
    import numpy as np
    lib = lib or load()
    rx = np.ascontiguousarray(rx, dtype=np.float32)
    floats = n_groups * GROUP * n_var * (1 if mod_type == 1 else 2) // max(mod_type, 1)
    if rx.size != floats:
        raise ValueError("%s: rx has %d floats, %d groups of mod_type %d take %d" % (fn_name, rx.size, n_groups, mod_type, floats))
    out = np.empty(n_groups * GROUP * n_var // (2 if packed else 1), dtype=np.uint8 if packed else np.int8)
    rc = getattr(lib, fn_name)(n_var, n_check, interleave, rx.ctypes.data, n_groups, mod_type, scale, out.ctypes.data)
    if rc != 0:
        raise ValueError("%s failed: %d" % (fn_name, rc))
    return out


def demap_host(n_var, n_check, interleave, rx, n_groups, mod_type, scale, lib=None):
    return _demap_host("lnsfaid_demap_host", False, n_var, n_check, interleave, rx, n_groups, mod_type, scale, lib)


def demap_packed_host(n_var, n_check, interleave, rx, n_groups, mod_type, scale, lib=None):
    return _demap_host("lnsfaid_demap_packed_host", True, n_var, n_check, interleave, rx, n_groups, mod_type, scale, lib)


class Decoder:

    def __init__(self, code50, cfg, device=0, max_groups=64, lib=None):
        self.lib = lib or load()
        self.code50 = code50
        self.ctx = C.c_void_p()
        rc = self.lib.lnsfaid_create(C.byref(self.ctx), C.byref(code50.code), C.byref(cfg), device, max_groups)
        if rc != 0:
            raise RuntimeError("lnsfaid_create failed: %d (%s; hip: %s)" % (
                rc, self.lib.lnsfaid_strerror(rc).decode(), self.lib.lnsfaid_last_hip_error().decode()))

    def _check(self, rc, what):
        if rc != 0:
            raise RuntimeError("%s failed: %d (%s; hip: %s)" % (
                what, rc, self.lib.lnsfaid_strerror(rc).decode(), self.lib.lnsfaid_last_hip_error().decode()))

    def set_cfg(self, cfg):
        self._check(self.lib.lnsfaid_set_cfg(self.ctx, C.byref(cfg)), "lnsfaid_set_cfg")

    def decode(self, fix_input, n_groups):
        import numpy as np
        N = self.code50.N
        assert fix_input.dtype == np.int8 and fix_input.size == n_groups * GROUP * N and fix_input.flags.c_contiguous
        out = np.empty(n_groups * GROUP * N, dtype=np.int8)
        stats = np.zeros((n_groups, 2), dtype=np.int32)
        self._check(self.lib.lnsfaid_decode(self.ctx, fix_input.ctypes.data, n_groups, out.ctypes.data,
                                            stats.ctypes.data), "lnsfaid_decode")
        return out, stats

    def set_early_stop(self, rule):
        self._check(self.lib.lnsfaid_set_early_stop(self.ctx, rule), "lnsfaid_set_early_stop")

    def early_stop(self):
        return self.lib.lnsfaid_early_stop(self.ctx)

    def decode_codewords(self, fix_input, n_groups, with_stats=True):
        import numpy as np
        N = self.code50.N
        assert fix_input.dtype == np.int8 and fix_input.size == n_groups * GROUP * N and fix_input.flags.c_contiguous
        out = np.empty(n_groups * GROUP * N, dtype=np.int8)
        cw = np.zeros((n_groups * GROUP, 3), dtype=np.int32) if with_stats else None
        self._check(self.lib.lnsfaid_decode_codewords(self.ctx, fix_input.ctypes.data, n_groups, out.ctypes.data,
                                                      cw.ctypes.data if with_stats else None), "lnsfaid_decode_codewords")
        return out, cw

    def decode_codewords_device(self, d_fix_ptr, n_groups, d_out_ptr, d_cw_stats_ptr=None):
        self._check(self.lib.lnsfaid_decode_codewords_device(self.ctx, d_fix_ptr, n_groups, d_out_ptr, d_cw_stats_ptr),
                    "lnsfaid_decode_codewords_device")

    def decode_device(self, d_fix_ptr, n_groups, d_out_ptr, d_stats_ptr=None):
        self._check(self.lib.lnsfaid_decode_device(self.ctx, d_fix_ptr, n_groups, d_out_ptr, d_stats_ptr),
                    "lnsfaid_decode_device")

    def count_errors(self, decoded, input_bits, n_groups):
        out = (C.c_uint64 * 4)()
        ip = input_bits.ctypes.data if input_bits is not None else None
        self._check(self.lib.lnsfaid_count_errors(self.ctx, decoded.ctypes.data, ip, n_groups, out), "lnsfaid_count_errors")
        return list(out)

    def count_errors_device(self, d_decoded_ptr, d_input_ptr, n_groups):
        out = (C.c_uint64 * 4)()
        self._check(self.lib.lnsfaid_count_errors_device(self.ctx, d_decoded_ptr, d_input_ptr, n_groups, out),
                    "lnsfaid_count_errors_device")
        return list(out)

    def decode_packed(self, llr4, n_groups):
        import numpy as np
        N = self.code50.N
        assert llr4.dtype == np.uint8 and llr4.size == n_groups * GROUP * N // 2 and llr4.flags.c_contiguous
        out = np.empty(n_groups * GROUP * N // 32, dtype=np.uint32)
        stats = np.zeros((n_groups, 2), dtype=np.int32)
        self._check(self.lib.lnsfaid_decode_packed(self.ctx, llr4.ctypes.data, n_groups, out.ctypes.data, stats.ctypes.data),
                    "lnsfaid_decode_packed")
        return out, stats

    def decode_codewords_packed(self, llr4, n_groups, with_stats=True):
        import numpy as np
        N = self.code50.N
        assert llr4.dtype == np.uint8 and llr4.size == n_groups * GROUP * N // 2 and llr4.flags.c_contiguous
        out = np.empty(n_groups * GROUP * N // 32, dtype=np.uint32)
        cw = np.zeros((n_groups * GROUP, 3), dtype=np.int32) if with_stats else None
        self._check(self.lib.lnsfaid_decode_codewords_packed(self.ctx, llr4.ctypes.data, n_groups, out.ctypes.data,
                                                             cw.ctypes.data if with_stats else None), "lnsfaid_decode_codewords_packed")
        return out, cw

    def decode_packed_device(self, d_llr4_ptr, n_groups, d_bits_ptr, d_stats_ptr=None):
        self._check(self.lib.lnsfaid_decode_packed_device(self.ctx, d_llr4_ptr, n_groups, d_bits_ptr, d_stats_ptr),
                    "lnsfaid_decode_packed_device")

    def decode_codewords_packed_device(self, d_llr4_ptr, n_groups, d_bits_ptr, d_cw_stats_ptr=None):
        self._check(self.lib.lnsfaid_decode_codewords_packed_device(self.ctx, d_llr4_ptr, n_groups, d_bits_ptr, d_cw_stats_ptr),
                    "lnsfaid_decode_codewords_packed_device")

    def count_errors_packed(self, bits, msg, n_groups):
        out = (C.c_uint64 * 4)()
        mp = msg.ctypes.data if msg is not None else None
        self._check(self.lib.lnsfaid_count_errors_packed(self.ctx, bits.ctypes.data, mp, n_groups, out), "lnsfaid_count_errors_packed")
        return list(out)

    def count_errors_packed_device(self, d_bits_ptr, d_msg_ptr, n_groups):
        out = (C.c_uint64 * 4)()
        self._check(self.lib.lnsfaid_count_errors_packed_device(self.ctx, d_bits_ptr, d_msg_ptr, n_groups, out),
                    "lnsfaid_count_errors_packed_device")
        return list(out)

    def demap_device(self, d_rx_ptr, n_groups, mod_type, scale, d_fix_ptr):
        self._check(self.lib.lnsfaid_demap_device(self.ctx, d_rx_ptr, n_groups, mod_type, scale, d_fix_ptr), "lnsfaid_demap_device")

    def demap_packed_device(self, d_rx_ptr, n_groups, mod_type, scale, d_llr4_ptr):
        self._check(self.lib.lnsfaid_demap_packed_device(self.ctx, d_rx_ptr, n_groups, mod_type, scale, d_llr4_ptr),
                    "lnsfaid_demap_packed_device")

    def encode(self, info, n_groups):
        import numpy as np
        K, N = self.code50.K, self.code50.N
        assert info.dtype == np.int8 and info.size == n_groups * GROUP * K and info.flags.c_contiguous
        out = np.empty(n_groups * GROUP * N, dtype=np.int8)
        self._check(self.lib.lnsfaid_encode(self.ctx, info.ctypes.data, n_groups, out.ctypes.data), "lnsfaid_encode")
        return out

    def encode_device(self, d_in_ptr, n_groups, d_out_ptr):
        self._check(self.lib.lnsfaid_encode_device(self.ctx, d_in_ptr, n_groups, d_out_ptr), "lnsfaid_encode_device")

    def random_frames(self, keys):
        buf = (C.c_uint64 * len(keys))(*[int(k) for k in keys])
        self._check(self.lib.lnsfaid_frontend_random_frames(self.ctx, buf, len(keys)), "lnsfaid_frontend_random_frames")

    def comm_init(self, n_ranks, rank, comm_id):
        self._check(self.lib.lnsfaid_comm_init(self.ctx, n_ranks, rank, comm_id), "lnsfaid_comm_init")

    def allreduce_counters(self, counters):
        buf = (C.c_uint64 * 4)(*[int(c) for c in counters])
        self._check(self.lib.lnsfaid_allreduce_counters(self.ctx, buf), "lnsfaid_allreduce_counters")
        return list(buf)

    def select_kernel(self, rows_per_lane):
        self._check(self.lib.lnsfaid_select_kernel(self.ctx, rows_per_lane), "lnsfaid_select_kernel")

    def rows_per_lane(self):
        return self.lib.lnsfaid_kernel_rows_per_lane(self.ctx)

    def select_waves(self, waves_per_codeword):
        self._check(self.lib.lnsfaid_select_waves(self.ctx, waves_per_codeword), "lnsfaid_select_waves")

    def kernel_waves(self):
        return self.lib.lnsfaid_kernel_waves(self.ctx)

    def select_message_store(self, where):
        self._check(self.lib.lnsfaid_select_message_store(self.ctx, where), "lnsfaid_select_message_store")

    def message_store(self):
        return self.lib.lnsfaid_message_store(self.ctx)

    def select_zero_shift(self, mode):
        self._check(self.lib.lnsfaid_select_zero_shift(self.ctx, mode), "lnsfaid_select_zero_shift")

    def zero_shift_groups(self, n_layers=32):
        zg = (C.c_int32 * n_layers)()
        on = self.lib.lnsfaid_zero_shift_groups(self.ctx, zg, n_layers)
        self._check(min(on, 0), "lnsfaid_zero_shift_groups")
        return on == 1, list(zg)

    def kernel_residency(self):
        wg, lim = C.c_int32(), C.c_int32()
        self._check(self.lib.lnsfaid_kernel_residency(self.ctx, C.byref(wg), C.byref(lim)), "lnsfaid_kernel_residency")
        return wg.value, lim.value

    def kernel_time(self, reset=False):
        ms = C.c_double()
        n = C.c_uint64()
        self._check(self.lib.lnsfaid_kernel_time(self.ctx, C.byref(ms), C.byref(n), 1 if reset else 0), "lnsfaid_kernel_time")
        return ms.value, n.value

    def close(self):
        if self.ctx:
            self.lib.lnsfaid_destroy(self.ctx)
            self.ctx = C.c_void_p()

    def __del__(self):
        try:
            self.close()
        except Exception:
            pass
```

Before: 77.17.

## Add static fully unrolled 50G-PON layer kernel with compile-time circulant tables

Adds a decode kernel specialised for the 50G-PON base matrix, with all 12 layers unrolled and each layer's column-block offsets and degrees taken from compile-time constants. The kernel is chosen by default whenever the runtime code matches the built-in table. This removes the per-edge OR of column bases into LDS addresses and the runtime degree handling, folding the column offsets into the LDS instruction's immediate offset. The cost is a code-specific kernel with larger code size and more register pressure, and the match check has to hold for the fast path to run.

```diff
diff --git a/include/lnsfaid.h b/include/lnsfaid.h
--- a/include/lnsfaid.h
+++ b/include/lnsfaid.h
@@ -174,6 +174,8 @@
 
 #define LNSFAID_ZERO_SHIFT_ON 1
 #define LNSFAID_ZERO_SHIFT_OFF 2
+#define LNSFAID_ZERO_SHIFT_LOOP 3
+#define LNSFAID_ZERO_SHIFT_STATIC 4
 int lnsfaid_select_zero_shift(lnsfaid_ctx* ctx, int32_t mode);
 int lnsfaid_zero_shift_groups(const lnsfaid_ctx* ctx, int32_t* groups, int32_t n);
 int lnsfaid_code_zero_shift_order(const lnsfaid_code* code, int32_t* groups, int32_t* order);
diff --git a/mod-interleaveavx_multithreads-faid_amd/csrc/lnsfaid_capi.hip b/mod-interleaveavx_multithreads-faid_amd/csrc/lnsfaid_capi.hip
--- a/mod-interleaveavx_multithreads-faid_amd/csrc/lnsfaid_capi.hip
+++ b/mod-interleaveavx_multithreads-faid_amd/csrc/lnsfaid_capi.hip
@@ -33,6 +33,9 @@
 extern "C" int lf_decode4z_inst(int deg, int zg);
 extern "C" const void* lf_decode4z_func(int method);
 extern "C" hipError_t lf_launch_decode4z(int method, const LfKernelArgs* args, size_t lds_bytes, hipStream_t stream);
+extern "C" int lf_decode4s_matches(const LfDevCode* code);
+extern "C" const void* lf_decode4s_func(int method);
+extern "C" hipError_t lf_launch_decode4s(int method, const LfKernelArgs* args, size_t lds_bytes, hipStream_t stream);
 extern "C" const void* lf_decode5_func(int method);
 extern "C" int lf_decode5_threads(void);
 extern "C" hipError_t lf_launch_decode5(int method, const LfKernelArgs* args, size_t lds_bytes, hipStream_t stream);
@@ -120,6 +123,7 @@
     int waves_per_cw = 0;
     int msg_store = 0;
     int zero_shift = 0;
+    mutable int static_code = -1;
     struct LfCombiner* comb = nullptr;
     int comb_slot = -1;
     const void* checked_fn[4] = {};
@@ -425,7 +429,7 @@
     if (const char* e = getenv("LNSFAID_MSG_STORE"))
         ctx->msg_store = (e[0] == 'h') ? LNSFAID_MSG_HBM : ((e[0] == 'r') ? LNSFAID_MSG_REGISTERS : 0);
     if (const char* e = getenv("LNSFAID_ZERO_SHIFT"))
-        ctx->zero_shift = (e[0] == 'o' && e[1] == 'f') ? LNSFAID_ZERO_SHIFT_OFF : 0;
+        ctx->zero_shift = (e[0] == 'o' && e[1] == 'f') ? LNSFAID_ZERO_SHIFT_OFF : (e[0] == 'l' ? LNSFAID_ZERO_SHIFT_LOOP : 0);
     g_live_contexts.fetch_add(1, std::memory_order_relaxed);
     const int rc = create_impl(ctx, code, cfg);
     if (rc) { lnsfaid_destroy(ctx); return rc; }
@@ -526,10 +530,21 @@
 }
 static bool use_zero_shift(const lnsfaid_ctx* ctx) { return ctx->zero_shift != LNSFAID_ZERO_SHIFT_OFF && zero_shift_possible(ctx); }
 
+static bool static_layers_possible(const lnsfaid_ctx* ctx)
+{
+    if (ctx->static_code < 0) ctx->static_code = lf_decode4s_matches(&ctx->hcode);
+    return ctx->static_code == 1 && zero_shift_possible(ctx) && lf_decode4s_func(ctx->hcfg.method);
+}
+static bool use_static_layers(const lnsfaid_ctx* ctx)
+{
+    return use_zero_shift(ctx) && ctx->zero_shift != LNSFAID_ZERO_SHIFT_LOOP && static_layers_possible(ctx);
+}
+
 extern "C" int lnsfaid_select_zero_shift(lnsfaid_ctx* ctx, int32_t mode)
 {
-    if (!ctx || mode < 0 || mode > LNSFAID_ZERO_SHIFT_OFF) return LNSFAID_E_INVAL;
-    if (mode == LNSFAID_ZERO_SHIFT_ON && !zero_shift_possible(ctx)) return LNSFAID_E_INVAL;
+    if (!ctx || mode < 0 || mode > LNSFAID_ZERO_SHIFT_STATIC) return LNSFAID_E_INVAL;
+    if ((mode == LNSFAID_ZERO_SHIFT_ON || mode == LNSFAID_ZERO_SHIFT_LOOP) && !zero_shift_possible(ctx)) return LNSFAID_E_INVAL;
+    if (mode == LNSFAID_ZERO_SHIFT_STATIC && !static_layers_possible(ctx)) return LNSFAID_E_INVAL;
     ctx->zero_shift = mode;
     return LNSFAID_OK;
 }
@@ -539,7 +554,7 @@
     if (!ctx || n < 0 || (n > 0 && !groups)) return LNSFAID_E_INVAL;
     const bool on = use_zero_shift(ctx);
     for (int br = 0; br < n; ++br) groups[br] = (on && br < ctx->hcode.nbr) ? layer_zero_groups(ctx, br) : 0;
-    return on ? 1 : 0;
+    return on ? (use_static_layers(ctx) ? 2 : 1) : 0;
 }
 
 extern "C" int lnsfaid_code_zero_shift_order(const lnsfaid_code* code, int32_t* groups, int32_t* order)
@@ -583,7 +598,7 @@
     }
     if (use_zero_shift(ctx)) {
         *threads = lf_decode4_threads();
-        return lf_decode4z_func(ctx->hcfg.method);
+        return use_static_layers(ctx) ? lf_decode4s_func(ctx->hcfg.method) : lf_decode4z_func(ctx->hcfg.method);
     }
     if (use_kernel4(ctx)) {
         *threads = lf_decode4_threads();
@@ -755,6 +770,7 @@
             HIP_TRY(hipEventRecord(ctx->ev_chain[j], ctx->stream));
             if (packed) HIP_TRY(lf_launch_decode4p(ctx->hcfg.method, ctx->hcfg.ef, use_msg_registers(ctx) ? 1 : 0, &a, ctx->lds_bytes, ctx->stream));
             else if (use_kernel5(ctx)) HIP_TRY(lf_launch_decode5(ctx->hcfg.method, &a, ctx->lds_bytes, ctx->stream));
+            else if (use_static_layers(ctx)) HIP_TRY(lf_launch_decode4s(ctx->hcfg.method, &a, ctx->lds_bytes, ctx->stream));
             else if (use_zero_shift(ctx)) HIP_TRY(lf_launch_decode4z(ctx->hcfg.method, &a, ctx->lds_bytes, ctx->stream));
             else if (use_kernel4(ctx)) HIP_TRY(lf_launch_decode4(ctx->hcfg.method, ctx->hcfg.ef, use_msg_registers(ctx) ? 1 : 0, &a, ctx->lds_bytes, ctx->stream));
             else HIP_TRY(lf_launch_decode(ctx->hcfg.method, ctx->hcfg.uniform_w, &a, ctx->lds_bytes, ctx->stream));
diff --git a/mod-interleaveavx_multithreads-faid_amd/csrc/lnsfaid_gpon_base.h b/mod-interleaveavx_multithreads-faid_amd/csrc/lnsfaid_gpon_base.h
--- /dev/null
+++ b/mod-interleaveavx_multithreads-faid_amd/csrc/lnsfaid_gpon_base.h
@@ -0,0 +1,24 @@
+#ifndef LNSFAID_GPON_BASE_H
+#define LNSFAID_GPON_BASE_H
+
+#define LNSFAID_GPON_BLOCK_ROWS 12
+#define LNSFAID_GPON_MAX_DEG 23
+
+#define LNSFAID_GPON_ROW_DEG { 23, 22, 23, 23, 23, 23, 23, 23, 23, 23, 23, 23 }
+
+#define LNSFAID_GPON_BASE { \
+     { {0,80}, {3,60}, {4,169}, {6,11}, {8,143}, {11,222}, {13,59}, {15,218}, {18,178}, {24,105}, {27,19}, {30,126}, {34,211}, {40,247}, {42,255}, {45,85}, {52,246}, {53,94}, {59,242}, {64,129}, {66,19}, {67,58}, {68,27} }, \
+     { {1,0}, {3,0}, {5,0}, {7,0}, {9,0}, {11,0}, {13,0}, {15,0}, {17,0}, {18,0}, {20,0}, {24,0}, {27,0}, {32,0}, {36,0}, {39,0}, {43,0}, {47,0}, {52,0}, {56,0}, {60,0}, {67,0} }, \
+     { {1,91}, {3,74}, {5,237}, {6,202}, {9,201}, {10,136}, {12,178}, {14,239}, {16,183}, {19,217}, {21,232}, {25,169}, {32,129}, {33,60}, {39,19}, {40,76}, {46,77}, {50,2}, {54,101}, {57,217}, {61,48}, {67,172}, {68,42} }, \
+     { {0,105}, {3,87}, {5,43}, {7,165}, {9,180}, {11,80}, {12,227}, {14,221}, {16,77}, {19,0}, {24,16}, {29,252}, {31,96}, {33,0}, {38,17}, {44,219}, {47,198}, {48,165}, {53,36}, {58,171}, {63,228}, {67,39}, {68,234} }, \
+     { {1,170}, {2,250}, {5,195}, {6,139}, {9,135}, {11,92}, {13,147}, {15,1}, {20,13}, {23,98}, {26,142}, {30,225}, {36,23}, {37,108}, {44,0}, {46,0}, {51,135}, {56,121}, {57,0}, {63,0}, {66,46}, {67,242}, {68,228} }, \
+     { {1,46}, {3,37}, {5,49}, {6,150}, {8,65}, {11,177}, {12,144}, {14,70}, {16,95}, {19,221}, {23,192}, {25,128}, {28,214}, {34,51}, {38,100}, {41,19}, {44,235}, {52,4}, {55,251}, {58,109}, {64,140}, {67,193}, {68,241} }, \
+     { {0,137}, {2,104}, {4,238}, {7,228}, {9,225}, {10,247}, {13,191}, {15,177}, {17,255}, {22,192}, {27,51}, {32,195}, {34,0}, {37,172}, {43,219}, {46,236}, {49,136}, {53,0}, {57,159}, {60,10}, {65,5}, {67,25}, {68,94} }, \
+     { {1,118}, {2,15}, {4,93}, {7,228}, {9,78}, {11,16}, {12,0}, {14,48}, {16,0}, {20,62}, {22,0}, {25,0}, {30,0}, {36,112}, {38,0}, {45,0}, {49,0}, {50,0}, {55,22}, {61,0}, {62,0}, {67,120}, {68,192} }, \
+     { {1,208}, {2,0}, {4,0}, {6,0}, {8,0}, {10,0}, {13,251}, {14,0}, {17,44}, {18,123}, {23,0}, {26,0}, {31,0}, {35,0}, {40,0}, {43,153}, {48,0}, {51,0}, {55,0}, {65,0}, {66,0}, {67,16}, {68,0} }, \
+     { {0,0}, {3,123}, {5,41}, {6,191}, {8,211}, {10,217}, {12,243}, {14,97}, {16,252}, {21,0}, {28,0}, {31,41}, {35,29}, {37,0}, {42,0}, {47,193}, {49,145}, {54,0}, {61,140}, {62,46}, {65,58}, {67,202}, {68,215} }, \
+     { {0,209}, {2,252}, {4,39}, {7,159}, {8,69}, {10,37}, {12,134}, {15,201}, {16,49}, {21,104}, {26,129}, {29,157}, {33,222}, {41,139}, {42,39}, {48,203}, {50,94}, {56,194}, {59,3}, {62,43}, {63,153}, {67,207}, {68,109} }, \
+     { {0,53}, {2,93}, {4,216}, {7,57}, {8,9}, {10,130}, {13,130}, {15,238}, {22,144}, {28,162}, {29,0}, {35,175}, {39,145}, {41,0}, {45,36}, {51,91}, {54,22}, {58,0}, {59,0}, {60,212}, {64,0}, {67,69}, {68,88} }, \
+}
+
+#endif
diff --git a/mod-interleaveavx_multithreads-faid_amd/csrc/lnsfaid_kernel4s.hip b/mod-interleaveavx_multithreads-faid_amd/csrc/lnsfaid_kernel4s.hip
--- /dev/null
+++ b/mod-interleaveavx_multithreads-faid_amd/csrc/lnsfaid_kernel4s.hip
@@ -0,0 +1,224 @@
+#include <hip/hip_runtime.h>
+
+#define LF4_MAIN_STEP main_step4s
+#include "lnsfaid_rows4.h"
+#include "lnsfaid_static50.h"
+
+static_assert(SW50_LAYERS == LF4_RM_LAYERS, "one register of every message vector per layer");
+
+extern "C" int lf_decode4s_matches(const LfDevCode* code)
+{
+    constexpr Sw50Code k = sw50_build();
+    if (!code || code->nbr != SW50_LAYERS) return 0;
+    for (int br = 0; br < SW50_LAYERS; ++br) {
+        if (code->deg[br] != k.layer[br].deg) return 0;
+        for (int j = 0; j < k.layer[br].deg; ++j) {
+            if (code->zs4tab[br][j] != k.layer[br].s4[j] || code->zcbtab[br][j] != k.layer[br].cb256[j]) return 0;
+            if (code->zsbplain[br][j] != ((k.layer[br].cb256[j] << 16) | k.layer[br].s4[j])) return 0;
+        }
+    }
+    return 1;
+}
+
+template <int METHOD, int BR>
+__device__ __forceinline__ void layer4s(const LfDevCode* gc, SwRegs& R, const SwLds& lds, const SwParams& p, const SwK& K, int lane, bool fresh,
+                                        const uint32_t* sP, bool have_par, bool lme, uint32_t& tabv)
+{
+    typedef Sw50Tab<BR> Tab;
+    asm volatile("; lf4s layer %1" : "+v"(lane) : "n"(BR));
+    uint32_t tabn = 0u;
+    if (BR + 1 < SW50_LAYERS) tabn = gc->zsbplain[BR + 1][lane & 31];
+    uint32_t rowpar = 0;
+    if (have_par) {
+#pragma unroll
+        for (int k = 0; k < 4; ++k) {
+            const uint32_t wv = sP[BR * 8 + 2 * k + (lane >> 5)];
+            rowpar |= ((wv >> (lane & 31)) & 1u) ? (0xffu << (8 * k)) : 0u;
+        }
+    }
+    Tab tab;
+    tab.sbv = tabv;
+    const SwRow cur = regs_get(R, BR);
+    SwRow st = sw_layer_step<METHOD, Tab::DEG>(lds, tab, p, K, (uint32_t)lane, Tab::DEG, cur, fresh, rowpar, lme);
+    asm volatile("" : "+v"(st.x[0]), "+v"(st.x[1]), "+v"(st.x[2]), "+v"(st.cw), "+v"(st.pa[0]), "+v"(st.pa[1]));
+    __builtin_amdgcn_sched_barrier(0);
+    regs_put(R, BR, st);
+    __builtin_amdgcn_sched_barrier(0);
+    tabv = tabn;
+}
+
+template <int METHOD, bool ERA, bool RM>
+__device__ __forceinline__ void main_step4s(CCode c, CCfg f, const LfDevCode* gc, SwRow* __restrict__ rows, SwRegs& R, int lane, int it, const uint32_t* sP,
+                                            bool have_par, bool lme, uint32_t era_plane)
+{
+    static_assert(RM && !ERA, "built for the messages-in-registers, non-erasing instances only");
+    (void)c; (void)rows; (void)era_plane;
+    it = __builtin_amdgcn_readfirstlane(it);
+    const SwK K = sw_consts((uint32_t)it);
+    const bool fresh = (it == 1);
+    const int rem = f->max_iter - it;
+    const int itx = (it >= 1 && it <= 5) ? it - 1 : 5;
+    SwParams p;
+    p.lut_lo = f->lut_lo[itx][0]; p.lut_hi = f->lut_hi[itx][0];
+    p.ef_lo = f->lut_ef_lo[itx][0]; p.ef_hi = f->lut_ef_hi[itx][0];
+    p.f1 = f->factor_1; p.f2 = f->factor_2;
+    p.window = rem <= f->floor_iter_thresh;
+    p.ef_tables = f->ef >= 1;
+    if (LF4_OMS(METHOD)) sw_oms_tables(p);
+    const SwLds lds = SwLds();
+    uint32_t tabv = gc->zsbplain[0][lane & 31];
+    __builtin_amdgcn_sched_barrier(0);
+    asm volatile("; lf4s layers begin");
+#define LF4S_LAYER(BR) layer4s<METHOD, BR>(gc, R, lds, p, K, lane, fresh, sP, have_par, lme, tabv);
+    LF4S_LAYER(0) LF4S_LAYER(1) LF4S_LAYER(2) LF4S_LAYER(3) LF4S_LAYER(4) LF4S_LAYER(5)
+    LF4S_LAYER(6) LF4S_LAYER(7) LF4S_LAYER(8) LF4S_LAYER(9) LF4S_LAYER(10) LF4S_LAYER(11)
+#undef LF4S_LAYER
+    asm volatile("; lf4s layers end");
+}
+
+#define LF4_ON_FRONT prog >= kmax
+#define LF4_CLEAN_STOPS(t) prog >= kmax && !group_passed(a.live, g, prog, t)
+#define LF4_ON_STOP(t) if (RM && prog >= 2) regs_store(R, g_rows, c->nbr, t);
+#define LF4_ON_PASS(t) publish_pass(a.live, cw, prog, t);
+
+template <int METHOD>
+__global__ __launch_bounds__(LF_T4, 2) void lnsfaid_decode4s_kernel(LfKernelArgs a)
+{
+    constexpr bool RM = true, EF2 = false;
+    extern __shared__ __align__(16) unsigned char smem[];
+    CCode c = (CCode)a.code;
+    CCfg f = (CCfg)a.cfg;
+    const int tid = (int)threadIdx.x;
+    const int cw = (int)blockIdx.x;
+    const int N = c->n_var, M = c->n_check, K = c->k_info, nw = c->n_words, pw = c->p_words;
+    uint32_t* sHard0 = (uint32_t*)smem;
+    uint32_t* sHard2 = (uint32_t*)smem + nw;
+    uint32_t* sHard = (uint32_t*)(smem + lf_lds_off_hard(N));
+    uint32_t* sP = (uint32_t*)(smem + lf_lds_off_p(N, nw));
+    int* sStat = (int*)(smem + lf_lds_off_stat(N, nw, pw));
+    int* sRed = sStat + LNSFAID_GROUP;
+
+    const int max_iter = f->max_iter, max_bf = f->max_bf;
+    const int t_bf0 = max_iter + 1;
+    const int t_end = t_bf0 + max_bf;
+
+    const int g = cw >> 5, lane_in_group = cw & 31;
+    const int sv = a.status_cur ? a.status_cur[g * LNSFAID_GROUP + (tid & 31)] : 0;
+    const int my_status = __builtin_amdgcn_readlane(sv, lane_in_group);
+    if (my_status & LF_DONE) {
+        if (tid == 0) a.status_next[cw] = my_status;
+        return;
+    }
+    if (tid == LNSFAID_GROUP) sRed[LF_ZERO_SLOT] = 0;
+    int kmax;
+    {
+        int v = sv & LF_PROG_MASK;
+        v = imax(v, __builtin_amdgcn_update_dpp(0, v, 0x111, 0xf, 0xf, false));
+        v = imax(v, __builtin_amdgcn_update_dpp(0, v, 0x112, 0xf, 0xf, false));
+        v = imax(v, __builtin_amdgcn_update_dpp(0, v, 0x114, 0xf, 0xf, false));
+        v = imax(v, __builtin_amdgcn_update_dpp(0, v, 0x118, 0xf, 0xf, false));
+        v = imax(v, __builtin_amdgcn_update_dpp(0, v, 0x142, 0xa, 0xf, false));
+        kmax = __builtin_amdgcn_readlane(v, 31);
+    }
+    const int all_same = __ballot(sv != my_status) == 0ull;
+    LF_WG_SYNC();
+    int prog = my_status & LF_PROG_MASK;
+
+    uint32_t* g_en = (uint32_t*)(a.st_en + (size_t)cw * (size_t)N);
+    SwRow* g_rows = (SwRow*)(a.st_rows + (size_t)cw * (size_t)(c->nbr * LF_T));
+    uint32_t* g_bits = a.st_bits + (size_t)cw * (size_t)(3 * nw);
+    int8_t* g_out = a.decoded + (size_t)cw * (size_t)N;
+
+    if (prog != 0 && prog == kmax && !all_same) {
+        if (tid == 0) { a.status_next[cw] = my_status; atomicAdd(a.remaining, 1u); }
+        return;
+    }
+
+    if (my_status != 0 && all_same) {
+        if (tid == 0) {
+            a.status_next[cw] = my_status | LF_DONE;
+            if (a.stats && lane_in_group == 0) {
+                lnsfaid_group_stats st;
+                st.iterations = prog <= max_iter ? prog - 1 : max_iter;
+                st.bf_iterations = prog <= max_iter ? 0 : prog - t_bf0;
+                a.stats[g] = st;
+            }
+        }
+        return;
+    }
+
+    bool in_bf = max_bf > 0 && prog >= t_bf0 && prog != 0;
+    LfLaneState ls = { 0, 0, 0, 0 };
+    SwRegs R;
+    if (RM) regs_clear(R);
+
+    if (prog == 0) {
+        LF4_STAGE_INPUT()
+        LF_WG_SYNC();
+        prog = 1;
+    } else if (!in_bf) {
+        copy_in<23>((uint32_t*)smem, g_en, N >> 2, tid);
+        if (RM && prog >= 2) regs_load(R, g_rows, c->nbr, tid);
+        LF_WG_SYNC();
+    } else {
+        copy_in<9>(sHard, g_bits, nw, tid);
+        copy_in<9>(sHard0, g_bits + nw, nw, tid);
+        copy_in<9>(sHard2, g_bits + 2 * nw, nw, tid);
+        ls = a.st_lane[cw];
+        LF_WG_SYNC();
+    }
+
+    bool parked = false;
+    uint32_t pA = 0, pB = 0;
+    if (!in_bf) {
+        LF4_LAYERED_LOOP()
+        LF4_ENTER_BF()
+    }
+    LF4_BF_LOOPS()
+
+    const bool finished = prog >= t_end;
+    if (finished) {
+        if (!in_bf) build_plane4<false>(c, sHard, 0, tid);
+        write_decoded(sHard, g_out, N, tid);
+        if (tid == 0) {
+            a.status_next[cw] = prog | LF_DONE;
+            if (a.stats && lane_in_group == 0) {
+                lnsfaid_group_stats st;
+                st.iterations = prog <= max_iter ? prog - 1 : max_iter;
+                st.bf_iterations = prog <= max_iter ? 0 : prog - t_bf0;
+                a.stats[g] = st;
+            }
+        }
+    } else {
+        if (!in_bf) {
+            copy_out<23>(g_en, (const uint32_t*)smem, N >> 2, tid);
+        } else {
+            copy_out<9>(g_bits, sHard, nw, tid);
+            copy_out<9>(g_bits + nw, sHard0, nw, tid);
+            copy_out<9>(g_bits + 2 * nw, sHard2, nw, tid);
+            if (tid == 0) a.st_lane[cw] = ls;
+        }
+        write_decoded(sHard, g_out, N, tid);
+        if (tid == 0) { a.status_next[cw] = prog; atomicAdd(a.remaining, 1u); }
+    }
+}
+
+extern "C" const void* lf_decode4s_func(int method)
+{
+    switch (method) {
+    case 1: return (const void*)lnsfaid_decode4s_kernel<1>;
+    case 2: return (const void*)lnsfaid_decode4s_kernel<2>;
+    case 3: return (const void*)lnsfaid_decode4s_kernel<3>;
+    case 4: return (const void*)lnsfaid_decode4s_kernel<4>;
+    case 5: return (const void*)lnsfaid_decode4s_kernel<5>;
+    default: return nullptr;
+    }
+}
+
+extern "C" hipError_t lf_launch_decode4s(int method, const LfKernelArgs* args, size_t lds_bytes, hipStream_t stream)
+{
+    const void* fn = lf_decode4s_func(method);
+    if (!fn) return hipErrorInvalidValue;
+    void* kargs[] = { (void*)args };
+    return hipLaunchKernel(fn, dim3((unsigned)args->n_cw), dim3(LF_T4), kargs, lds_bytes, stream);
+}
diff --git a/mod-interleaveavx_multithreads-faid_amd/csrc/lnsfaid_static50.h b/mod-interleaveavx_multithreads-faid_amd/csrc/lnsfaid_static50.h
--- /dev/null
+++ b/mod-interleaveavx_multithreads-faid_amd/csrc/lnsfaid_static50.h
@@ -0,0 +1,77 @@
+#ifndef LNSFAID_STATIC50_H
+#define LNSFAID_STATIC50_H
+
+#include "lnsfaid_gpon_base.h"
+#include "lnsfaid_swar.h"
+
+#define SW50_LAYERS LNSFAID_GPON_BLOCK_ROWS
+
+struct Sw50Layer {
+    int deg, nz;
+    uint32_t s4[SW_MAX_DEG];
+    uint32_t cb256[SW_MAX_DEG];
+};
+struct Sw50Code {
+    Sw50Layer layer[SW50_LAYERS];
+};
+
+constexpr Sw50Code sw50_build()
+{
+    struct Circ { int cb, shift; };
+    constexpr int deg[SW50_LAYERS] = LNSFAID_GPON_ROW_DEG;
+    constexpr Circ base[SW50_LAYERS][LNSFAID_GPON_MAX_DEG] = LNSFAID_GPON_BASE;
+    Sw50Code c = {};
+    for (int br = 0; br < SW50_LAYERS; ++br) {
+        int n = 0;
+        for (int zero = 1; zero >= 0; --zero)
+            for (int j = 0; j < deg[br]; ++j)
+                if ((base[br][j].shift == 0) == (zero != 0)) {
+                    c.layer[br].s4[n] = (uint32_t)base[br][j].shift << 2;
+                    c.layer[br].cb256[n] = (uint32_t)base[br][j].cb << 8;
+                    ++n;
+                }
+        c.layer[br].deg = n;
+        int nz = 0;
+        while (nz < n && c.layer[br].s4[nz] == 0u) ++nz;
+        c.layer[br].nz = nz;
+    }
+    return c;
+}
+
+template <int BR>
+struct Sw50Tab {
+    static_assert(BR >= 0 && BR < SW50_LAYERS, "layer of the 50G-PON code");
+    static constexpr Sw50Layer L = sw50_build().layer[BR];
+    static constexpr int DEG = L.deg, NZ = L.nz;
+    uint32_t sbv;
+    SW_MFN uint32_t s4(int j) const { return L.s4[j]; }
+    SW_MFN uint32_t cb256(int j) const { return L.cb256[j]; }
+    SW_MFN uint32_t sb_dyn4(uint32_t idx4) const
+    {
+#if SW_DEV
+        return (uint32_t)__builtin_amdgcn_ds_bpermute((int)idx4, (int)sbv);
+#else
+        return (L.cb256[idx4 >> 2] << 16) | L.s4[idx4 >> 2];
+#endif
+    }
+};
+template <int BR>
+struct SwTabStatic<Sw50Tab<BR>> {
+    static constexpr bool value = true;
+    static constexpr int nz = Sw50Tab<BR>::NZ;
+};
+
+constexpr bool sw50_check()
+{
+    constexpr Sw50Code c = sw50_build();
+    int zeros = 0, edges = 0;
+    for (int br = 0; br < SW50_LAYERS; ++br) {
+        for (int j = 0; j < c.layer[br].deg; ++j)
+            if (c.layer[br].cb256[j] + 255u > 0xffffu) return false;
+        zeros += c.layer[br].nz; edges += c.layer[br].deg;
+    }
+    return zeros == 69 && edges == 275;
+}
+static_assert(sw50_check(), "50G-PON base matrix: 275 circulants, 69 of them identities, block columns inside the offset field");
+
+#endif
diff --git a/mod-interleaveavx_multithreads-faid_amd/csrc/lnsfaid_swar.h b/mod-interleaveavx_multithreads-faid_amd/csrc/lnsfaid_swar.h
--- a/mod-interleaveavx_multithreads-faid_amd/csrc/lnsfaid_swar.h
+++ b/mod-interleaveavx_multithreads-faid_amd/csrc/lnsfaid_swar.h
@@ -186,16 +186,16 @@
 struct SwLds {
     typedef __attribute__((address_space(3))) uint32_t lds_u32;
     typedef __attribute__((address_space(3))) uint8_t lds_u8;
-    SW_FN uint32_t rd32(uint32_t a) const { return *(const lds_u32*)(size_t)a; }
-    SW_FN void wr32(uint32_t a, uint32_t v) const { *(lds_u32*)(size_t)a = v; }
+    SW_FN uint32_t rd32(uint32_t a, uint32_t off = 0u) const { return *(const lds_u32*)(size_t)(a + off); }
+    SW_FN void wr32(uint32_t a, uint32_t v, uint32_t off = 0u) const { *(lds_u32*)(size_t)(a + off) = v; }
     SW_FN uint32_t rd8(uint32_t a) const { return *(const lds_u8*)(size_t)a; }
     SW_FN void wr8(uint32_t a, uint32_t v) const { *(lds_u8*)(size_t)a = (uint8_t)v; }
 };
 #else
 struct SwLds {
     uint8_t* base;
-    uint32_t rd32(uint32_t a) const { return (uint32_t)base[a] | ((uint32_t)base[a + 1] << 8) | ((uint32_t)base[a + 2] << 16) | ((uint32_t)base[a + 3] << 24); }
-    void wr32(uint32_t a, uint32_t v) const { base[a] = (uint8_t)v; base[a + 1] = (uint8_t)(v >> 8); base[a + 2] = (uint8_t)(v >> 16); base[a + 3] = (uint8_t)(v >> 24); }
+    uint32_t rd32(uint32_t a, uint32_t off = 0u) const { a += off; return (uint32_t)base[a] | ((uint32_t)base[a + 1] << 8) | ((uint32_t)base[a + 2] << 16) | ((uint32_t)base[a + 3] << 24); }
+    void wr32(uint32_t a, uint32_t v, uint32_t off = 0u) const { a += off; base[a] = (uint8_t)v; base[a + 1] = (uint8_t)(v >> 8); base[a + 2] = (uint8_t)(v >> 16); base[a + 3] = (uint8_t)(v >> 24); }
     uint32_t rd8(uint32_t a) const { return base[a]; }
     void wr8(uint32_t a, uint32_t v) const { base[a] = (uint8_t)v; }
 };
@@ -387,6 +387,12 @@
 };
 #define SW_OWN(j) (WAVES == 1 || (((j) & 1) == WAVE))
 
+template <class Tab>
+struct SwTabStatic {
+    static constexpr bool value = false;
+    static constexpr int nz = 0;
+};
+
 template <int METHOD, int DEG, bool ERA = false, int WAVES = 1, int WAVE = 0, int ZG = 0, class Tab, class Xch = SwNoXch>
 SW_FN SwRow sw_layer_step(const SwLds& lds, const Tab& tab, const SwParams& p, const SwK& K, uint32_t lane, int deg, SwRow cur, bool fresh,
                           uint32_t rowpar, bool lme, uint32_t era_edges = 0u, uint32_t era_plane = 0u, const Xch& xch = Xch())
@@ -394,7 +400,9 @@
     static_assert(WAVES == 1 || !ERA, "the erasing variant is built for one wave per codeword only");
     static_assert(!ERA || METHOD == 2, "the erasure exists in Decode_FAID only");
     static_assert(ZG == 0 || (DEG > 0 && WAVES == 1 && !ERA && SW_ILP * ZG <= DEG), "rotation-free groups: per-degree, one-wave, non-erasing instances");
-    constexpr int NZ = SW_ILP * ZG;
+    constexpr bool STATIC = SwTabStatic<Tab>::value;
+    static_assert(!STATIC || (ZG == 0 && DEG > 0 && WAVES == 1 && !ERA && SwTabStatic<Tab>::nz <= DEG), "static table view: per-degree, one-wave, non-erasing instances");
+    constexpr int NZ = STATIC ? SwTabStatic<Tab>::nz : SW_ILP * ZG;
     constexpr int NJ = DEG > 0 ? DEG : SW_MAX_DEG;
     constexpr bool MINSUM = SW_MINSUM(METHOD);
     constexpr bool QUADS = WAVES == 1 && SW_ILP == 4 && DEG > 0;
@@ -435,21 +443,23 @@
 #pragma unroll
     for (int j = 0; j < NJ; ++j) {
         if (j < NZ) {
-            ad[j] = tid4 | cbj[j];
+            ad[j] = STATIC ? tid4 : tid4 | cbj[j];
         } else if ((DEG > 0 || j < deg) && SW_OWN(j)) {
             const uint32_t x4 = tid4 + s4j[j];
 #if SW_DEV
             uint32_t a;
-            asm("v_and_or_b32 %0, %1, %2, %3" : "=v"(a) : "v"(x4), "v"(cfc), "s"(cbj[j]));
-#else
-            const uint32_t a = (x4 & cfc) | cbj[j];
+            if (STATIC) a = x4 & cfc;
+            else asm("v_and_or_b32 %0, %1, %2, %3" : "=v"(a) : "v"(x4), "v"(cfc), "s"(cbj[j]));
+#else
+            const uint32_t a = STATIC ? x4 & cfc : (x4 & cfc) | cbj[j];
 #endif
             ad[j] = a; rq[j] = x4 >> 8;
         }
     }
+#define SW_COL(j) (STATIC ? cbj[j] : 0u)
 #pragma unroll
     for (int j = 0; j < NJ; ++j)
-        if ((DEG > 0 || j < deg) && SW_OWN(j)) ld[j] = lds.rd32(ad[j]);
+        if ((DEG > 0 || j < deg) && SW_OWN(j)) ld[j] = lds.rd32(ad[j], SW_COL(j));
     SW_SCHED_FENCE();
 #pragma unroll
     for (int j0 = 0; j0 < NJ; j0 += SW_ILP) {
@@ -459,7 +469,7 @@
         SW_EDGES(x_[g] = (j & 7) ? cur.x[j >> 3] >> (j & 7) : cur.x[j >> 3];)
         SW_EDGES(s_[g] = sw_bitop3<SW_TT_ANDOR>(x_[g], c01, c0642);)
         SW_EDGES(k_[g] = sw_perm(kt_hi, kt_lo, s_[g]);)
-        if (j0 < NZ) { _Pragma("unroll") for (int g = SW_ILP - 1; g >= 0; --g) tb[j0 + g] = r_[g] + k_[g]; }
+        if ((j0 + SW_ILP < NJ ? j0 + SW_ILP : NJ) <= NZ) { _Pragma("unroll") for (int g = SW_ILP - 1; g >= 0; --g) if (j0 + g < NJ) tb[j0 + g] = r_[g] + k_[g]; }
         else { SW_EDGES(tb[j] = r_[g] + k_[g];) }
         if (ERA) {
             SW_EDGES(x_[g] &= c01;)
@@ -596,7 +606,7 @@
 #define SW_PASS2_STORE(J0, EN)                                                                                       \
     {                                                                                                                \
         const int j0 = (J0);                                                                                         \
-        SW_EDGES(lds.wr32(ad[j], EN[g]);)                                                                            \
+        SW_EDGES(lds.wr32(ad[j], EN[g], SW_COL(j));)                                                                 \
     }
     uint32_t en0[SW_ILP], en1[SW_ILP];
     SW_PASS2_ARITH(0, en0)
@@ -652,6 +662,7 @@
 #undef SW_EDGES
 #undef SW_PASS2_ARITH
 #undef SW_PASS2_STORE
+#undef SW_COL
     if (WAVES == 2) {
         if (WAVE == 1) { xch.put(0, ns[0]); xch.put(1, ns[1]); xch.put(2, ns[2]); }
         xch.barrier();
diff --git a/mod-interleaveavx_multithreads-faid_amd/csrc/lnsfaid_tables.c b/mod-interleaveavx_multithreads-faid_amd/csrc/lnsfaid_tables.c
--- a/mod-interleaveavx_multithreads-faid_amd/csrc/lnsfaid_tables.c
+++ b/mod-interleaveavx_multithreads-faid_amd/csrc/lnsfaid_tables.c
@@ -1,29 +1,18 @@
 #include "lnsfaid.h"
 #include <string.h>
 
+#include "lnsfaid_gpon_base.h"
+
 #define GPON_Z 256
-#define GPON_BLOCK_ROWS 12
+#define GPON_BLOCK_ROWS LNSFAID_GPON_BLOCK_ROWS
 #define GPON_BLOCK_COLS 69
-#define GPON_MAX_DEG 23
+#define GPON_MAX_DEG LNSFAID_GPON_MAX_DEG
 
 typedef struct { int16_t cb; int16_t shift; } gpon_circ;
 
-static const int gpon_row_deg[GPON_BLOCK_ROWS] = { 23, 22, 23, 23, 23, 23, 23, 23, 23, 23, 23, 23 };
+static const int gpon_row_deg[GPON_BLOCK_ROWS] = LNSFAID_GPON_ROW_DEG;
 
-static const gpon_circ gpon_base[GPON_BLOCK_ROWS][GPON_MAX_DEG] = {
-     { {0,80}, {3,60}, {4,169}, {6,11}, {8,143}, {11,222}, {13,59}, {15,218}, {18,178}, {24,105}, {27,19}, {30,126}, {34,211}, {40,247}, {42,255}, {45,85}, {52,246}, {53,94}, {59,242}, {64,129}, {66,19}, {67,58}, {68,27} },
-     { {1,0}, {3,0}, {5,0}, {7,0}, {9,0}, {11,0}, {13,0}, {15,0}, {17,0}, {18,0}, {20,0}, {24,0}, {27,0}, {32,0}, {36,0}, {39,0}, {43,0}, {47,0}, {52,0}, {56,0}, {60,0}, {67,0} },
-     { {1,91}, {3,74}, {5,237}, {6,202}, {9,201}, {10,136}, {12,178}, {14,239}, {16,183}, {19,217}, {21,232}, {25,169}, {32,129}, {33,60}, {39,19}, {40,76}, {46,77}, {50,2}, {54,101}, {57,217}, {61,48}, {67,172}, {68,42} },
-     { {0,105}, {3,87}, {5,43}, {7,165}, {9,180}, {11,80}, {12,227}, {14,221}, {16,77}, {19,0}, {24,16}, {29,252}, {31,96}, {33,0}, {38,17}, {44,219}, {47,198}, {48,165}, {53,36}, {58,171}, {63,228}, {67,39}, {68,234} },
-     { {1,170}, {2,250}, {5,195}, {6,139}, {9,135}, {11,92}, {13,147}, {15,1}, {20,13}, {23,98}, {26,142}, {30,225}, {36,23}, {37,108}, {44,0}, {46,0}, {51,135}, {56,121}, {57,0}, {63,0}, {66,46}, {67,242}, {68,228} },
-     { {1,46}, {3,37}, {5,49}, {6,150}, {8,65}, {11,177}, {12,144}, {14,70}, {16,95}, {19,221}, {23,192}, {25,128}, {28,214}, {34,51}, {38,100}, {41,19}, {44,235}, {52,4}, {55,251}, {58,109}, {64,140}, {67,193}, {68,241} },
-     { {0,137}, {2,104}, {4,238}, {7,228}, {9,225}, {10,247}, {13,191}, {15,177}, {17,255}, {22,192}, {27,51}, {32,195}, {34,0}, {37,172}, {43,219}, {46,236}, {49,136}, {53,0}, {57,159}, {60,10}, {65,5}, {67,25}, {68,94} },
-     { {1,118}, {2,15}, {4,93}, {7,228}, {9,78}, {11,16}, {12,0}, {14,48}, {16,0}, {20,62}, {22,0}, {25,0}, {30,0}, {36,112}, {38,0}, {45,0}, {49,0}, {50,0}, {55,22}, {61,0}, {62,0}, {67,120}, {68,192} },
-     { {1,208}, {2,0}, {4,0}, {6,0}, {8,0}, {10,0}, {13,251}, {14,0}, {17,44}, {18,123}, {23,0}, {26,0}, {31,0}, {35,0}, {40,0}, {43,153}, {48,0}, {51,0}, {55,0}, {65,0}, {66,0}, {67,16}, {68,0} },
-     { {0,0}, {3,123}, {5,41}, {6,191}, {8,211}, {10,217}, {12,243}, {14,97}, {16,252}, {21,0}, {28,0}, {31,41}, {35,29}, {37,0}, {42,0}, {47,193}, {49,145}, {54,0}, {61,140}, {62,46}, {65,58}, {67,202}, {68,215} },
-     { {0,209}, {2,252}, {4,39}, {7,159}, {8,69}, {10,37}, {12,134}, {15,201}, {16,49}, {21,104}, {26,129}, {29,157}, {33,222}, {41,139}, {42,39}, {48,203}, {50,94}, {56,194}, {59,3}, {62,43}, {63,153}, {67,207}, {68,109} },
-     { {0,53}, {2,93}, {4,216}, {7,57}, {8,9}, {10,130}, {13,130}, {15,238}, {22,144}, {28,162}, {29,0}, {35,175}, {39,145}, {41,0}, {45,36}, {51,91}, {54,22}, {58,0}, {59,0}, {60,212}, {64,0}, {67,69}, {68,88} },
-};
+static const gpon_circ gpon_base[GPON_BLOCK_ROWS][GPON_MAX_DEG] = LNSFAID_GPON_BASE;
 
 int lnsfaid_code_50gpon(lnsfaid_code* code, uint16_t* pos_vn, int32_t* deg3, int32_t* deg_rows3)
 {
diff --git a/mod-interleaveavx_multithreads-faid_amd/pyabi.py b/mod-interleaveavx_multithreads-faid_amd/pyabi.py
--- a/mod-interleaveavx_multithreads-faid_amd/pyabi.py
+++ b/mod-interleaveavx_multithreads-faid_amd/pyabi.py
@@ -6,7 +6,7 @@
 
 GROUP = 32
 MSG_REGISTERS, MSG_HBM = 1, 2
-ZERO_SHIFT_ON, ZERO_SHIFT_OFF = 1, 2
+ZERO_SHIFT_ON, ZERO_SHIFT_OFF, ZERO_SHIFT_LOOP, ZERO_SHIFT_STATIC = 1, 2, 3, 4
 STOP_GROUP, STOP_CODEWORD = 0, 1
 
 
@@ -404,7 +404,12 @@
         zg = (C.c_int32 * n_layers)()
         on = self.lib.lnsfaid_zero_shift_groups(self.ctx, zg, n_layers)
         self._check(min(on, 0), "lnsfaid_zero_shift_groups")
-        return on == 1, list(zg)
+        return on >= 1, list(zg)
+
+    def static_layers(self):
+        on = self.lib.lnsfaid_zero_shift_groups(self.ctx, None, 0)
+        self._check(min(on, 0), "lnsfaid_zero_shift_groups")
+        return on == 2
 
     def kernel_residency(self):
         wg, lim = C.c_int32(), C.c_int32()
```

Result: faster. 80.22, median of 6 (+4.0%).
